# LikeLy-Journey/SegmenTron

Measured on AMD Instinct MI355X. Metric: images/sec fwd+bwd DeepLabv3+_xception65 @1025x2049, higher is better.
Workload: dtype bf16; 1 GPU; DeepLabv3+_xception65 train step (fwd + CE loss + bwd + SGD) @1025x2049, batch 2/GPU (BASELINE.json configs[2]); global_batch=2, bn=BN, parallelism=dp1, full_size=True

## Files before the change

include/segmentron_hip.h:

```cpp
#ifndef SEGMENTRON_HIP_H
#define SEGMENTRON_HIP_H
#ifdef __cplusplus
extern "C" {
#endif

const char* seg_last_error(void);
int seg_version(void);

int seg_conv_gemm_fwd(int dtype, const void* x, long ldx, int N, int Hi, int Wi, int C,
                      const void* w, int O, int KH, int KW, int stride, int pad, int dil,
                      int pro_mode, const float* pro_scale, const float* pro_shift,
                      const float* bias, void* y, long ldy, int Ho, int Wo, int out_H, int out_W,
                      int out_s, float* stat_partial, const void* ep_x, long ldep,
                      const float* ep_c0, const float* ep_c1, int tconv, void* stream);
int seg_conv_gemm_tiles_m(int N, int Ho, int Wo);

int seg_conv_gemm_wgrad(int dtype, const void* x, long ldx, int N, int Hi, int Wi, int C,
                        const void* dy, long lddy, int Ho, int Wo, int O, int KH, int KW,
                        int stride, int pad, int dil, int pro_mode, const float* pro_scale,
                        const float* pro_shift, float* partial, int splits, void* stream);
int seg_conv_gemm_stat_rows(int dtype, int N, int Ho, int Wo, int C, int O, int KH, int KW,
                            int stride, int pad, int dil, int tconv, int has_bias, int pro_mode);
int seg_conv_gemm_wgrad_splits(int dtype, int N, int Ho, int Wo, int C, int O, int KH, int KW,
                               int stride, int pad, int dil, int pro_mode);

int seg_dwconv3x3(int dtype, int mode, const void* x, long ldx, int N, int Hi, int Wi, int C,
                  const float* w9c, int w_layout, int stride, int dil, int pro_mode,
                  const float* pro_scale, const float* pro_shift, void* y, long ldy, int Ho, int Wo,
                  float* stat_partial, int grid_y, void* stream);
int seg_dwconv_grid_y(int dtype, int C, int N, int Ho, int Wo, int stride, int dil, int kind);
int seg_dwconv3x3_wgrad_finalize(const float* partial, int R, int C, float* dw_c9, void* stream);
int seg_dwconv3x3_wgrad(int dtype, const void* x, long ldx, int N, int Hi, int Wi, int C,
                        const void* dy, long lddy, int Ho, int Wo, int stride, int dil,
                        int pro_mode, const float* pro_scale, const float* pro_shift,
                        float* partial, int grid_y, void* stream);

int seg_dwconv3x3_bwd_fused(int dtype, const void* dy, long lddy, const void* x, long ldx, int N,
                            int H, int W, int C, const float* w9c, int w_layout, int dil,
                            int pro_mode, const float* pro_scale, const float* pro_shift, void* g,
                            long ldg, float* partial_w, float* partial_bn, int grid_y,
                            void* stream);
int seg_dwconv3x3_bwd_fused_add_ok(int dil);
int seg_dwconv3x3_bwd_fused_add(int dtype, const void* dy, long lddy, const void* x, long ldx, int N,
                                int H, int W, int C, const float* w9c, int w_layout, int pro_mode,
                                const float* pro_scale, const float* pro_shift, const void* res,
                                long ldr, void* g, long ldg, float* partial_w, float* partial_bn,
                                int grid_y, void* stream);

int seg_colsum(const float* in, long R, int L, double* out_d, float* out_f, double* ws,
               void* stream);
int seg_colsum_count(const float* in, long R, int L, double* out_d, double count, double* ws,
                     void* stream);
int seg_bn_finalize(const double* sums, double count, const double* count_dev,
                    const float* gamma, const float* beta, float eps, float momentum, float* running_mean, float* running_var,
                    float* mean, float* invstd, float* scale, float* shift, int C,
                    const float* mean_offset, void* stream);
int seg_bn_finalize_p(const float* partial, long R, double count, const float* gamma,
                      const float* beta, float eps, float momentum, float* running_mean,
                      float* running_var, float* mean, float* invstd, float* scale, float* shift,
                      int C, const float* mean_offset, double* ws, void* stream);
int seg_bn_finalize_small(int dtype, const void* y, long ldy, long M, int C, const float* gamma,
                          const float* beta, float eps, float momentum, float* running_mean,
                          float* running_var, float* mean, float* invstd, float* scale,
                          float* shift, const float* mean_offset, void* stream);
int seg_bn_moments_small(int dtype, const void* y, long ldy, long M, int C, double* moments,
                         void* stream);
int seg_bn_finalize_small_sync(void* p2p, int dtype, const void* y, long ldy, long M, int C,
                               const float* gamma, const float* beta, float eps, float momentum,
                               float* running_mean, float* running_var, float* mean, float* invstd,
                               float* scale, float* shift, const float* mean_offset,
                               double* count_out, void* stream);
int seg_sum_n(int dtype, int n, const void* const* xs, const long* lds, void* y, long ldy, long M,
              int C, void* stream);
int seg_bn_eval_affine(const float* gamma, const float* beta, const float* rm, const float* rv,
                       float eps, float* scale, float* shift, int C, void* stream);
int seg_bn_eval_affine_multi(int n, const float* const* gamma, const float* const* beta,
                             const float* const* rm, const float* const* rv, const float* eps,
                             float* const* out, const int* C, void* stream);
int seg_bn_apply(int dtype, const void* x, long ldx, int mode_x, const float* sx, const float* tx,
                 const void* r, long ldr, int mode_r, const float* sr, const float* tr,
                 const float* chan_mul, long rows_per_n, const void* elem_mul, long ldm,
                 int post_relu, void* y, long ldy, long M, int C, void* stream);
int seg_bn_bwd_grid_y(int dtype, int C, long M);
int seg_ew_geom_query(int dtype, int C, long M, int what);
int seg_bn_bwd_reduce(int dtype, const void* g, long ldg, const void* x, long ldx, int mode,
                      const float* scale, const float* shift, const float* chan_mul,
                      long rows_per_n, const void* elem_mul, long ldm, long M, int C,
                      float* partial, int grid_y, void* stream);
int seg_bn_bwd_small(int dtype, const void* g, long ldg, const void* x, long ldx, void* dx,
                     long lddx, long M, int C, int mode, const float* scale, const float* shift,
                     const float* mean, const float* invstd, const float* gamma,
                     const float* chan_mul, long rows_per_n, const void* elem_mul, long ldm,
                     double count, int training, float* dgamma, float* dbeta, void* stream);
int seg_bn_bwd_finalize(const double* sums, double count, const double* count_dev,
                        const float* mean, const float* invstd, const float* gamma, float* dgamma, float* dbeta, float* c0, float* c1,
                        int C, void* stream);
int seg_bn_bwd_finalize_s(const double* sums, double count, const double* count_dev,
                          const float* mean, const float* invstd, const float* gamma, float* dgamma,
                          float* dbeta, float* c0, float* c1, int C, double grad_scale, void* stream);
int seg_bn_bwd_finalize_p(const float* partial, long R, double count, const float* mean,
                          const float* invstd, const float* gamma, float* dgamma, float* dbeta,
                          float* c0, float* c1, int C, double* ws, void* stream);
int seg_dw_bwd_finalize(const float* partial_bn, int Rb, double count, const float* mean,
                        const float* invstd, const float* gamma, float* dgamma, float* dbeta,
                        float* c0, float* c1, const float* partial_w, int Rw, float* dw_c9, int C,
                        void* stream);
int seg_bn_bwd_apply(int dtype, const void* g, long ldg, const void* x, long ldx, int mode,
                     const float* scale, const float* shift, const float* c0, const float* c1,
                     const float* chan_mul, long rows_per_n, const void* elem_mul, long ldm,
                     void* dx, long lddx, long M, int C, void* stream);

int seg_gn_chunks(long HW);
int seg_gn_moments(int dtype, const void* u, long ldu, const void* v, long ldv, int N, long HW,
                   int C, float* partial, void* stream);
int seg_gn_fwd_finalize(const float* partial, int N, long HW, int C, int G, const float* gamma,
                        const float* beta, double eps, float* mean_rstd, float* coef,
                        void* stream);
int seg_gn_bwd_finalize(const float* partial, int N, long HW, int C, int G,
                        const float* mean_rstd, const float* gamma, float* coef, float* contrib,
                        void* stream);
int seg_gn_affine(int dtype, const void* u, long ldu, const void* v, long ldv, const float* coef,
                  void* out, long ldo, int N, long HW, int C, void* stream);

int seg_fold_weights(int dtype, const float* W, const float* scale, const float* shift, void* Wp,
                     void* WpT, float* bprime, int O, int C, void* stream);
int seg_fold_bwd_rows(int O);
int seg_fold_bwd_reduce(const float* W, const float* dWp, int splits, const float* scale,
                        const float* shift, const float* db, float* dW, float* dsdt, int O, int C,
                        void* stream);
int seg_fold_bwd_finalize(const float* dsdt, int rows, double count, const double* count_dev,
                          const float* mean, const float* invstd, const float* gamma, const float* scale, float* dgamma, float* dbeta,
                          float* c0, float* c1, int C, void* stream);
int seg_fold_bwd_finalize_s(const float* dsdt, int rows, double count, const double* count_dev,
                            const float* mean, const float* invstd, const float* gamma,
                            const float* scale, float* dgamma, float* dbeta, float* c0, float* c1,
                            int C, double grad_scale, void* stream);

int seg_maxpool_fwd(int dtype, const void* x, long ldx, int N, int Hi, int Wi, int C, int k,
                    int stride, int pad, int pro_mode, const float* pro_scale,
                    const float* pro_shift, void* y, long ldy, int Ho, int Wo, void* idx,
                    void* stream);
int seg_maxpool_bwd(int dtype, void* gx, long ldgx, int N, int Hi, int Wi, int C, int k, int stride,
                    int pad, const void* gy, long ldgy, int Ho, int Wo, const void* idx,
                    void* stream);
int seg_adaptive_avgpool_chunks(int H, int W, int o);
int seg_adaptive_avgpool_partial(int dtype, const void* x, long ldx, int N, int H, int W, int C,
                                 int o, float* partial, int chunks, void* stream);
int seg_adaptive_avgpool_bwd(int dtype, void* gx, long ldgx, int N, int H, int W, int C, int o,
                             const void* gy, long ldgy, void* stream);

int seg_bilinear_fwd(int dtype, const void* x, long ldx, int N, int Hi, int Wi, int C,
                     int pro_mode, const float* pro_scale, const float* pro_shift,
                     const float* chan_mul, void* y, long ldy, int Ho, int Wo, int align_corners,
                     void* stream);
int seg_bilinear_bwd(int dtype, void* gx, long ldgx, int N, int Hi, int Wi, int C, const void* gy,
                     long ldgy, int Ho, int Wo, int align_corners, void* stream);
int seg_nearest_add(int dtype, const void* x, long ldx, int mode_x, const float* sx,
                    const float* tx, const void* r, long ldr, int mode_r, const float* sr,
                    const float* tr, int shift, int post_relu, void* y, long ldy, int N, int H,
                    int W, int C, void* stream);
int seg_nearest_sum_bwd(int dtype, const void* g, long ldg, int N, int H, int W, int C, int shift,
                        void* gr, long ldgr, void* stream);
int seg_upsample_to_nchw(int dtype, const void* x, long ldx, int N, int Hi, int Wi, int C,
                         float* out, int Ho, int Wo, int align_corners, void* stream);
int seg_upsample_to_nchw_bwd(int dtype, void* gx, long ldgx, int N, int Hi, int Wi, int C,
                             const float* gy, int Ho, int Wo, int align_corners, void* stream);
int seg_nchw_to_nhwc_pad(int dtype, const float* x, int N, int Cin, int H, int W, void* y,
                         void* stream);

int seg_upsample_ce_blocks(int N, int H, int W);
int seg_upsample_ce_fwd(int dtype, const void* lo, long ld, int N, int Hi, int Wi, int C,
                        const long* target, int H, int W, long ignore_index, int align_corners,
                        double* ws, float* loss_out, void* stream);
int seg_upsample_ce_bwd(int dtype, const void* lo, long ld, int N, int Hi, int Wi, int C,
                        const long* target, int H, int W, long ignore_index, int align_corners,
                        const float* loss_out, const float* grad_out, void* dlo, long lddlo,
                        void* stream);

int seg_point_sample(int dtype_x, const void* x, long sn, long sp, long sc, int N, int H, int W,
                     int C, const float* pts, int P, int nearest, int dtype_y, void* y, long ldy,
                     int col, void* stream);
int seg_point_sample_bwd_ws(int N, int H, int W, int P);
int seg_point_sample_bwd(int dtype_g, const void* g, long ldg, int col, const float* pts, int N,
                         int P, int H, int W, int C, int dtype_x, void* dx, long lddx, int* ws,
                         void* stream);
int seg_point_uncertainty(int dtype, const void* x, long sn, long sp, long sc, int N, int H, int W,
                          int C, const float* pts, int P, float* u, void* stream);
int seg_point_topk_ws(int N, long L);
int seg_point_topk(const float* keys, int N, long L, int K, long* idx, int* ws, void* stream);
int seg_point_coords(const float* over, const long* idx, int N, int L, int K, const float* cover,
                     int P, int H, int W, float* pts, void* stream);
int seg_point_scatter(int dtype_r, const void* rend, long ldr, const long* idx, int N, int P,
                      int C, float* y, long sn, long sp, long sc, void* stream);
int seg_point_resize(int dtype, const void* x, long sn, long sp, long sc, int N, int Hi, int Wi,
                     int C, float* y, int Ho, int Wo, int align_corners, void* stream);
int seg_point_ce_blocks(long R);
int seg_point_ce_fwd(int dtype, const void* x, long ldx, long R, int C, const long* target,
                     long ignore_index, double* ws, float* loss_out, void* stream);
int seg_point_ce_bwd(int dtype, const void* x, long ldx, long R, int C, const long* target,
                     long ignore_index, const float* loss_out, const float* grad_out, void* dx,
                     long lddx, void* stream);

int seg_dwconv3x3_s2_grid_y(int C, int N, int H, int W);
int seg_dwconv3x3_s2_bwd_fused(int dtype, const void* dy, long lddy, const void* x, long ldx, int N,
                               int H, int W, int C, const float* w_c9, int pro_mode,
                               const float* pro_scale, const float* pro_shift, void* g, long ldg,
                               float* partial_w, float* partial_bn, int grid_y, void* stream);

int seg_sgd_multi_tensor(int ntensors, const void* const* params, const void* const* grads,
                         const void* const* bufs, const long* numel, const int* group,
                         const float* lr_dev, const float* wd_dev, float momentum, int first,
                         void* stream);
int seg_pack_multi(int dtype, int njobs, const void* const* srcs, const void* const* dsts,
                   const int* O, const int* C, const int* transpose, void* stream);

int seg_metric_update_nchw(const float* logits, int N, int C, int H, int W, const long* target,
                           int nclass, long* counters, void* stream);
int seg_metric_update_upsample(int dtype, const void* lo, long ld, int N, int Hi, int Wi, int C,
                               const long* target, int H, int W, int align_corners, int nclass,
                               long* counters, void* stream);

int seg_cca_attention(int dtype, const void* q, long ldq, const void* k, long ldk, int N, int H,
                      int W, int C, float* att, void* stream);
int seg_cca_attention_bwd(int dtype, const void* dout, long lddo, const void* v, long ldv, int N,
                          int H, int W, int C, const float* att, const float* scale, float* de,
                          void* stream);
int seg_cca_map(int dtype, const float* wt, const void* b, long ldb, int N, int H, int W, int C,
                int transposed, const float* gamma, const void* res, long ldres, void* out,
                long ldo, void* raw, long ldraw, void* stream);

int seg_row_softmax(const void* e, int dt_in, long lde, void* a, int dt_out, long lda, long R,
                    int L, int Lp, float sign, void* stream);
int seg_row_softmax_bwd(const void* a, int dt_a, long lda, const void* g, int dt_g, long ldg,
                        void* de, int dt_out, long ldde, long R, int L, int Lp, float sign,
                        void* stream);
int seg_p2p_create(int rank, int world, long slot_bytes, void** handle_out);
int seg_p2p_ipc_handle(void* handle, void* out64);
int seg_p2p_connect(void* handle, const void* handles);
int seg_p2p_all_reduce_f64(void* handle, void* buf, int n, void* stream);
int seg_p2p_all_reduce_f32(void* handle, void* buf, int n, void* stream);
int seg_p2p_status(void* handle);
int seg_p2p_set_timeout(void* handle, double seconds);
int seg_p2p_destroy(void* handle);
int seg_bn_finalize_p_sync(void* p2p, const float* partial, long R, double local_count,
                           const float* gamma, const float* beta, float eps, float momentum,
                           float* running_mean, float* running_var, float* mean, float* invstd,
                           float* scale, float* shift, int C, const float* mean_offset,
                           double* count_out, double* ws, void* stream);
int seg_bn_bwd_finalize_p_sync(void* p2p, const float* partial, long R, const double* count_dev,
                               const float* mean, const float* invstd, const float* gamma,
                               float* dgamma, float* dbeta, float* c0, float* c1, int C,
                               double grad_scale, double* ws, void* stream);
int seg_dw_bwd_finalize_sync(void* p2p, const float* partial_bn, int Rb, const double* count_dev,
                             const float* mean, const float* invstd, const float* gamma,
                             float* dgamma, float* dbeta, float* c0, float* c1,
                             const float* partial_w, int Rw, float* dw_c9, int C,
                             double grad_scale, void* stream);
int seg_fold_bwd_finalize_sync(void* p2p, const float* dsdt, int rows, const double* count_dev,
                               const float* mean, const float* invstd, const float* gamma,
                               const float* scale, float* dgamma, float* dbeta, float* c0,
                               float* c1, int C, double grad_scale, void* stream);

#ifdef __cplusplus
}
#endif
#endif
```

segmentron_amd/csrc/dwconv.hip:

```cpp
#include "common.h"
#include "dwconv_tiled.h"
#include "dwconv_slide.h"
#include <cstdlib>
#include <type_traits>

namespace seg {

constexpr bool g_dw_row = true;

constexpr int DW_TW = 4;
constexpr int DW_THREADS = 256;
enum { MODE_FWD = 0, MODE_DGRAD = 1 };

struct DwArgs {
  const void* x;
  const float* w;
  void* y;
  const float* pro_scale;
  const float* pro_shift;
  float* stat_partial;
  long ldx, ldy;
  int N, Hi, Wi, C;
  int Ho, Wo;
  int stride, pad, dil;
  int pro_mode;
  int cvb_log2;
  int CV;
  long strips;
};

__device__ __forceinline__ int fast_div(int s, int d, float inv) {
  int q = (int)((float)s * inv);
  if (q * d > s) --q;
  if ((q + 1) * d <= s) ++q;
  return q;
}

template <int VEC>
__device__ __forceinline__ void dw_act(float* f, int mode, const float* sc, const float* sh) {
  if (mode & PRO_AFFINE) {
#pragma unroll
    for (int i = 0; i < VEC; ++i) f[i] = fmaf(f[i], sc[i], sh[i]);
  }
  if (mode & PRO_RELU) {
#pragma unroll
    for (int i = 0; i < VEC; ++i) f[i] = fmaxf(f[i], 0.f);
  }
  if (mode & PRO_CLAMP6) {
#pragma unroll
    for (int i = 0; i < VEC; ++i) f[i] = fminf(f[i], 6.f);
  }
}

template <typename T, int MODE>
__global__ __launch_bounds__(DW_THREADS, 2) void dwconv_kernel(const DwArgs a) {
  using V = Vec<T>;
  constexpr int VEC = V::N;
  extern __shared__ __attribute__((aligned(16))) float dw_smem[];
  const int tid = threadIdx.x;
  const int cvb = 1 << a.cvb_log2;
  const int cx = tid & (cvb - 1), sy = tid >> a.cvb_log2;
  const int spb = DW_THREADS >> a.cvb_log2;
  const int cv = blockIdx.x * cvb + cx;
  const bool cok = cv < a.CV;
  const int c0 = cok ? cv * VEC : 0;
  const T* __restrict__ X = reinterpret_cast<const T*>(a.x);
  T* __restrict__ Y = reinterpret_cast<T*>(a.y);
  const int WQ = (a.Wo + DW_TW - 1) / DW_TW;
  const float inv_wq = 1.0f / (float)WQ, inv_ho = 1.0f / (float)a.Ho;

  float sc[VEC], sh[VEC];
  if (a.pro_mode & PRO_AFFINE) {
    load_params<VEC>(a.pro_scale, c0, sc);
    load_params<VEC>(a.pro_shift, c0, sh);
  } else {
#pragma unroll
    for (int i = 0; i < VEC; ++i) { sc[i] = 1.f; sh[i] = 0.f; }
  }
  float ssum[VEC], ssq[VEC];
#pragma unroll
  for (int i = 0; i < VEC; ++i) ssum[i] = ssq[i] = 0.f;

  const int nstrips = (int)a.strips;
  for (int s = blockIdx.y * spb + sy; s < nstrips; s += gridDim.y * spb) {
    if (!cok) continue;
    const int t = fast_div(s, WQ, inv_wq);
    const int wq = s - t * WQ;
    const int n = fast_div(t, a.Ho, inv_ho);
    const int ho = t - n * a.Ho;
    const int w0 = wq * DW_TW;
    float acc[DW_TW][VEC];
#pragma unroll
    for (int j = 0; j < DW_TW; ++j)
#pragma unroll
      for (int i = 0; i < VEC; ++i) acc[j][i] = 0.f;

#pragma unroll
    for (int kh = 0; kh < 3; ++kh) {
      int hi;
      if (MODE == MODE_FWD) {
        hi = ho * a.stride - a.pad + kh * a.dil;
      } else {
        const int hn = ho + a.pad - kh * a.dil;
        if (hn < 0 || (hn % a.stride) != 0) continue;
        hi = hn / a.stride;
      }
      if (hi < 0 || hi >= a.Hi) continue;
      const long rowbase = ((long)n * a.Hi + hi) * a.Wi;
#pragma unroll
      for (int kw = 0; kw < 3; ++kw) {
        float wv[VEC];
        load_params<VEC>(a.w + (kh * 3 + kw) * a.C, c0, wv);
#pragma unroll
        for (int j = 0; j < DW_TW; ++j) {
          const int wo = w0 + j;
          int wi;
          bool ok = wo < a.Wo;
          if (MODE == MODE_FWD) {
            wi = wo * a.stride - a.pad + kw * a.dil;
          } else {
            const int wn = wo + a.pad - kw * a.dil;
            ok = ok && wn >= 0 && (wn % a.stride) == 0;
            wi = wn / a.stride;
          }
          ok = ok && wi >= 0 && wi < a.Wi;
          if (ok) {
            float f[VEC];
            V::unpack_raw(V::load_raw(X + (rowbase + wi) * a.ldx + c0), f);
            dw_act<VEC>(f, a.pro_mode, sc, sh);
#pragma unroll
            for (int i = 0; i < VEC; ++i) acc[j][i] = fmaf(f[i], wv[i], acc[j][i]);
          }
        }
      }
    }
    const long orow = ((long)n * a.Ho + ho) * a.Wo;
#pragma unroll
    for (int j = 0; j < DW_TW; ++j) {
      if (w0 + j < a.Wo) {
        V::store(Y + (orow + w0 + j) * a.ldy + c0, acc[j]);
#pragma unroll
        for (int i = 0; i < VEC; ++i) {
          ssum[i] += acc[j][i];
          ssq[i] += acc[j][i] * acc[j][i];
        }
      }
    }
  }

  if (a.stat_partial != nullptr) {
    float* mine = dw_smem + ((long)sy * cvb + cx) * 2 * VEC;
#pragma unroll
    for (int i = 0; i < VEC; ++i) {
      mine[i] = ssum[i];
      mine[VEC + i] = ssq[i];
    }
    __syncthreads();
    for (int e = tid; e < cvb * 2 * VEC; e += DW_THREADS) {
      float tot = 0.f;
      for (int r = 0; r < spb; ++r) tot += dw_smem[(long)r * cvb * 2 * VEC + e];
      const int lcx = e / (2 * VEC), k = e % (2 * VEC);
      const int which = k / VEC, ci = k % VEC;
      const int c = (blockIdx.x * cvb + lcx) * VEC + ci;
      if (c < a.C) a.stat_partial[((long)blockIdx.y * 2 + which) * a.C + c] = tot;
    }
  }
}

struct DwWgradArgs {
  const void* x;
  const void* dy;
  float* partial;
  const float* pro_scale;
  const float* pro_shift;
  long ldx, lddy;
  int N, Hi, Wi, C, Ho, Wo;
  int stride, pad, dil;
  int pro_mode;
  int cvb_log2, CV;
  long strips;
};

template <typename T>
__global__ __launch_bounds__(DW_THREADS) void dwconv_wgrad_kernel(const DwWgradArgs a) {
  constexpr int VEC = Vec<T>::N;
  extern __shared__ __attribute__((aligned(16))) float dw_smem[];
  const int tid = threadIdx.x;
  const int cvb = 1 << a.cvb_log2;
  const int cx = tid & (cvb - 1), sy = tid >> a.cvb_log2;
  const int spb = DW_THREADS >> a.cvb_log2;
  const int cv = blockIdx.x * cvb + cx;
  const bool cok = cv < a.CV;
  const int c0 = cok ? cv * VEC : 0;
  const T* __restrict__ X = reinterpret_cast<const T*>(a.x);
  const T* __restrict__ DY = reinterpret_cast<const T*>(a.dy);
  const int WQ = (a.Wo + DW_TW - 1) / DW_TW;
  const float inv_wq = 1.0f / (float)WQ, inv_ho = 1.0f / (float)a.Ho;

  float sc[VEC], sh[VEC];
  if (a.pro_mode & PRO_AFFINE) {
    load_params<VEC>(a.pro_scale, c0, sc);
    load_params<VEC>(a.pro_shift, c0, sh);
  } else {
#pragma unroll
    for (int i = 0; i < VEC; ++i) { sc[i] = 1.f; sh[i] = 0.f; }
  }
  float acc[9][VEC];
#pragma unroll
  for (int k = 0; k < 9; ++k)
#pragma unroll
    for (int i = 0; i < VEC; ++i) acc[k][i] = 0.f;

  const int nstrips = (int)a.strips;
  for (int s = blockIdx.y * spb + sy; s < nstrips; s += gridDim.y * spb) {
    if (!cok) continue;
    const int t = fast_div(s, WQ, inv_wq);
    const int wq = s - t * WQ;
    const int n = fast_div(t, a.Ho, inv_ho);
    const int ho = t - n * a.Ho;
    const int w0 = wq * DW_TW;
    const long orow = ((long)n * a.Ho + ho) * a.Wo;
    float g[DW_TW][VEC];
#pragma unroll
    for (int j = 0; j < DW_TW; ++j) {
      const int wc = min(w0 + j, a.Wo - 1);
      Vec<T>::unpack(ldg16(DY + (orow + wc) * a.lddy + c0), g[j]);
      const float keep = (w0 + j < a.Wo) ? 1.f : 0.f;
#pragma unroll
      for (int i = 0; i < VEC; ++i) g[j][i] *= keep;
    }
#pragma unroll
    for (int kh = 0; kh < 3; ++kh) {
      const int hi = ho * a.stride - a.pad + kh * a.dil;
      if (hi < 0 || hi >= a.Hi) continue;
      const long rowbase = ((long)n * a.Hi + hi) * a.Wi;
#pragma unroll
      for (int kw = 0; kw < 3; ++kw) {
#pragma unroll
        for (int j = 0; j < DW_TW; ++j) {
          const int wi = (w0 + j) * a.stride - a.pad + kw * a.dil;
          if (w0 + j < a.Wo && wi >= 0 && wi < a.Wi) {
            float f[VEC];
            Vec<T>::unpack(ldg16(X + (rowbase + wi) * a.ldx + c0), f);
            dw_act<VEC>(f, a.pro_mode, sc, sh);
#pragma unroll
            for (int i = 0; i < VEC; ++i)
              acc[kh * 3 + kw][i] = fmaf(f[i], g[j][i], acc[kh * 3 + kw][i]);
          }
        }
      }
    }
  }
#pragma unroll
  for (int k3 = 0; k3 < 3; ++k3) {
    float* mine = dw_smem + ((long)sy * cvb + cx) * 3 * VEC;
#pragma unroll
    for (int kk = 0; kk < 3; ++kk)
#pragma unroll
      for (int i = 0; i < VEC; ++i) mine[kk * VEC + i] = acc[k3 * 3 + kk][i];
    __syncthreads();
    for (int e = tid; e < cvb * 3 * VEC; e += DW_THREADS) {
      float tot = 0.f;
      for (int r = 0; r < spb; ++r) tot += dw_smem[(long)r * cvb * 3 * VEC + e];
      const int lcx = e / (3 * VEC), k = e % (3 * VEC);
      const int kk = k / VEC, ci = k % VEC;
      const int c = (blockIdx.x * cvb + lcx) * VEC + ci;
      if (c < a.C) a.partial[((long)blockIdx.y * 9 + k3 * 3 + kk) * a.C + c] = tot;
    }
    __syncthreads();
  }
}

struct DwBwdArgs {
  const void* dy; const void* x; void* g;
  const float* w;
  const float* pro_scale; const float* pro_shift;
  float* partial_w;
  float* partial_bn;
  long lddy, ldx, ldg;
  int N, H, W, C, dil, pro_mode, cvb_log2, CV;
  long strips;
};

template <typename T>
__global__ __launch_bounds__(DW_THREADS) void dwconv_bwd_fused_kernel(const DwBwdArgs a) {
  constexpr int VEC = HVec<T>::N;
  extern __shared__ __attribute__((aligned(16))) float dw_smem[];
  const int tid = threadIdx.x;
  const int cvb = 1 << a.cvb_log2;
  const int cx = tid & (cvb - 1), sy = tid >> a.cvb_log2;
  const int spb = DW_THREADS >> a.cvb_log2;
  const int cv = blockIdx.x * cvb + cx;
  const bool cok = cv < a.CV;
  const int c0 = cok ? cv * VEC : 0;
  const T* __restrict__ DY = reinterpret_cast<const T*>(a.dy);
  const T* __restrict__ X = reinterpret_cast<const T*>(a.x);
  T* __restrict__ G = reinterpret_cast<T*>(a.g);
  const int WQ = (a.W + DW_TW - 1) / DW_TW;
  const float inv_wq = 1.0f / (float)WQ, inv_h = 1.0f / (float)a.H;
  const int d = a.dil;

  float sc[VEC], sh[VEC];
  if (a.pro_mode & PRO_AFFINE) {
    load_params<VEC>(a.pro_scale, c0, sc);
    load_params<VEC>(a.pro_shift, c0, sh);
  } else {
#pragma unroll
    for (int i = 0; i < VEC; ++i) { sc[i] = 1.f; sh[i] = 0.f; }
  }
  float accw[9][VEC], s1[VEC], s2[VEC];
#pragma unroll
  for (int k = 0; k < 9; ++k)
#pragma unroll
    for (int i = 0; i < VEC; ++i) accw[k][i] = 0.f;
#pragma unroll
  for (int i = 0; i < VEC; ++i) s1[i] = s2[i] = 0.f;

  const int nstrips = (int)a.strips;
  for (int s = blockIdx.y * spb + sy; s < nstrips; s += gridDim.y * spb) {
    if (!cok) continue;
    const int t = fast_div(s, WQ, inv_wq);
    const int wq = s - t * WQ;
    const int n = fast_div(t, a.H, inv_h);
    const int h = t - n * a.H;
    const int w0 = wq * DW_TW;
    const long prow = ((long)n * a.H + h) * a.W;
    float xr[DW_TW][VEC], xa[DW_TW][VEC], g[DW_TW][VEC];
#pragma unroll
    for (int j = 0; j < DW_TW; ++j) {
      const int wc = min(w0 + j, a.W - 1);
      HVec<T>::load(X + (prow + wc) * a.ldx + c0, xr[j]);
      const float keep = (w0 + j < a.W) ? 1.f : 0.f;
#pragma unroll
      for (int i = 0; i < VEC; ++i) {
        xa[j][i] = xr[j][i];
        g[j][i] = 0.f;
      }
      dw_act<VEC>(xa[j], a.pro_mode, sc, sh);
#pragma unroll
      for (int i = 0; i < VEC; ++i) {
        xa[j][i] *= keep;
        xr[j][i] *= keep;
      }
    }
#pragma unroll
    for (int kh = 0; kh < 3; ++kh) {
      const int r = h + (1 - kh) * d;
      if (r < 0 || r >= a.H) continue;
      const long rowbase = ((long)n * a.H + r) * a.W;
#pragma unroll
      for (int kw = 0; kw < 3; ++kw) {
        float wv[VEC];
        load_params<VEC>(a.w + (kh * 3 + kw) * a.C, c0, wv);
#pragma unroll
        for (int j = 0; j < DW_TW; ++j) {
          const int c = w0 + j + (1 - kw) * d;
          if (w0 + j < a.W && c >= 0 && c < a.W) {
            float dyv[VEC];
            HVec<T>::load(DY + (rowbase + c) * a.lddy + c0, dyv);
#pragma unroll
            for (int i = 0; i < VEC; ++i) {
              g[j][i] = fmaf(dyv[i], wv[i], g[j][i]);
              accw[kh * 3 + kw][i] = fmaf(dyv[i], xa[j][i], accw[kh * 3 + kw][i]);
            }
          }
        }
      }
    }
#pragma unroll
    for (int j = 0; j < DW_TW; ++j) {
      if (w0 + j < a.W) {
        if (a.pro_mode & PRO_RELU) {
#pragma unroll
          for (int i = 0; i < VEC; ++i) {
            const bool on = xa[j][i] > 0.f && (!(a.pro_mode & PRO_CLAMP6) || xa[j][i] < 6.f);
            g[j][i] = on ? g[j][i] : 0.f;
          }
        }
#pragma unroll
        for (int i = 0; i < VEC; ++i) {
          s1[i] += g[j][i];
          s2[i] = fmaf(g[j][i], xr[j][i], s2[i]);
        }
        HVec<T>::store(G + (prow + w0 + j) * a.ldg + c0, g[j]);
      }
    }
  }
#pragma unroll
  for (int k3 = 0; k3 < 4; ++k3) {
    if (k3 == 3 && a.partial_bn == nullptr) break;
    float* mine = dw_smem + ((long)sy * cvb + cx) * 3 * VEC;
#pragma unroll
    for (int kk = 0; kk < 3; ++kk)
#pragma unroll
      for (int i = 0; i < VEC; ++i)
        mine[kk * VEC + i] = k3 < 3 ? accw[(k3 < 3 ? k3 : 0) * 3 + kk][i]
                                    : (kk == 0 ? s1[i] : (kk == 1 ? s2[i] : 0.f));
    __syncthreads();
    const int ncol = (k3 < 3 ? 3 : 2) * VEC;
    for (int e = tid; e < cvb * 3 * VEC; e += DW_THREADS) {
      const int lcx = e / (3 * VEC), k = e % (3 * VEC);
      if (k >= ncol) continue;
      float tot = 0.f;
      for (int r = 0; r < spb; ++r) tot += dw_smem[(long)r * cvb * 3 * VEC + e];
      const int kk = k / VEC, ci = k % VEC;
      const int c = (blockIdx.x * cvb + lcx) * VEC + ci;
      if (c < a.C) {
        if (k3 < 3) a.partial_w[((long)blockIdx.y * 9 + k3 * 3 + kk) * a.C + c] = tot;
        else a.partial_bn[((long)blockIdx.y * 2 + kk) * a.C + c] = tot;
      }
    }
    __syncthreads();
  }
}

static int pick_cvb_log2(int CV) {
  int best = 5;
  double bu = 0;
  for (int l = 5; l >= 3; --l) {
    const int b = 1 << l;
    const double u = (double)CV / (double)(((CV + b - 1) / b) * b);
    if (u > bu + 1e-9) { bu = u; best = l; }
  }
  return best;
}

}

extern "C" int seg_dwconv_grid_y(int dtype, int C, int N, int Ho, int Wo, int stride, int dil,
                                 int kind) {
  using namespace seg;
  const int tiled_stride = kind == 0 ? stride : 1;
  if ((kind == 0 || kind == 1) && dw_slide_supported(stride, dil, C))
    return dw_slide_rows(C, N, Ho, Wo);
  if ((kind == 0 || stride == 1) && dw_tiled_supported(tiled_stride, dil))
    return dw_tiled_grid_y(dtype, C, N, Ho, Wo, kind);
  if (kind == 0 && stride == 2 && dil == 1)
    return dw_tiled_s2_grid_y(dtype, C, N, Ho, Wo);
  if (g_dw_row && (kind == 0 || kind == 1) && dw_row_supported(stride, dil) && C % 4 == 0)
    return dw_row_grid_y(dtype, C, N, Ho, Wo, dil);
  const int vec = dtype == DT_BF16 ? 8 : 4;
  const int CV = C / vec;
  const int l = pick_cvb_log2(CV);
  const int spb = DW_THREADS >> l;
  const long strips = (long)N * Ho * ((Wo + DW_TW - 1) / DW_TW);
  const int gx = (CV + (1 << l) - 1) >> l;
  long gy = (strips + spb - 1) / spb;
  long cap = 1536 / gx;
  if (cap < 1) cap = 1;
  if (gy > cap) gy = cap;
  return (int)gy;
}
extern "C" int seg_dwconv3x3(int dtype, int mode, const void* x, long ldx, int N, int Hi, int Wi,
                             int C, const float* w9c, int w_layout, int stride, int dil, int pro_mode,
                             const float* pro_scale, const float* pro_shift, void* y, long ldy,
                             int Ho, int Wo, float* stat_partial, int grid_y, void* stream) {
  using namespace seg;
  const int vec = dtype == DT_BF16 ? 8 : 4;
  SEG_REQUIRE(dtype == DT_F32 || dtype == DT_BF16, "dwconv3x3: bad dtype %d", dtype);
  SEG_REQUIRE(C % vec == 0 && ldx % vec == 0 && ldy % vec == 0,
              "dwconv3x3: C/ldx/ldy must be multiples of %d", vec);
  SEG_REQUIRE(((pro_mode & PRO_AFFINE) == 0) || (pro_scale && pro_shift),
              "dwconv3x3: affine prologue without scale/shift");
  SEG_REQUIRE(mode == MODE_FWD || stat_partial == nullptr, "dwconv3x3: stats only in forward");
  SEG_REQUIRE(grid_y >= 1, "dwconv3x3: grid_y must be >= 1");
  if (mode == MODE_FWD && dw_slide_supported(stride, dil, C)) {
    SEG_REQUIRE(Ho == Hi && Wo == Wi, "dwconv3x3: stride 1 keeps the size");
    return launch_dw_slide_fwd(dtype, x, ldx, N, Hi, Wi, C, w9c, w_layout, pro_mode, pro_scale,
                               pro_shift, y, ldy, stat_partial, grid_y, (hipStream_t)stream);
  }
  if (mode == MODE_FWD && dw_tiled_supported(stride, dil)) {
    SEG_REQUIRE(Ho == Hi && Wo == Wi, "dwconv3x3: stride 1 keeps the size");
    return launch_dw_tiled(dtype, x, ldx, N, Hi, Wi, C, w9c, w_layout, dil, pro_mode, pro_scale,
                           pro_shift, y, ldy, stat_partial, grid_y, (hipStream_t)stream);
  }
  if (mode == MODE_FWD && stride == 2 && dil == 1) {
    SEG_REQUIRE(Ho == (Hi + 1) / 2 && Wo == (Wi + 1) / 2, "dwconv3x3: stride-2 output size");
    SEG_REQUIRE((long)N * Hi * Wi < (1L << 31), "dwconv3x3: tensor exceeds 32-bit pixel offsets");
    return launch_dw_tiled_s2(dtype, x, ldx, N, Hi, Wi, C, w9c, w_layout, pro_mode, pro_scale,
                              pro_shift, y, ldy, stat_partial, grid_y, (hipStream_t)stream);
  }
  SEG_REQUIRE(w_layout == 0, "dwconv3x3: the strip kernels take tap-major [9][C] weights");
  if (g_dw_row && mode == MODE_FWD && dw_row_supported(stride, dil) && C % 4 == 0) {
    SEG_REQUIRE(Ho == Hi && Wo == Wi, "dwconv3x3: stride 1 keeps the size");
    return launch_dw_row_fwd(dtype, x, ldx, N, Hi, Wi, C, w9c, dil, pro_mode, pro_scale, pro_shift,
                             y, ldy, stat_partial, grid_y, (hipStream_t)stream);
  }
  DwArgs a;
  a.x = x; a.w = w9c; a.y = y; a.pro_scale = pro_scale; a.pro_shift = pro_shift;
  a.stat_partial = stat_partial; a.ldx = ldx; a.ldy = ldy;
  a.N = N; a.Hi = Hi; a.Wi = Wi; a.C = C; a.Ho = Ho; a.Wo = Wo;
  a.stride = stride; a.pad = dil; a.dil = dil; a.pro_mode = pro_mode;
  const int kvec = vec;
  a.CV = C / kvec; a.cvb_log2 = pick_cvb_log2(a.CV);
  a.strips = (long)N * Ho * ((Wo + DW_TW - 1) / DW_TW);
  const int gx = (a.CV + (1 << a.cvb_log2) - 1) >> a.cvb_log2;
  SEG_REQUIRE(grid_y >= 1, "dwconv3x3: grid_y must be >= 1");
  const dim3 grid(gx, grid_y);
  const size_t lds = stat_partial ? (size_t)DW_THREADS * 2 * kvec * sizeof(float) : 0;
  hipStream_t st = (hipStream_t)stream;
  SEG_REQUIRE(a.strips < (1L << 31), "dwconv3x3: too many strips");
  SEG_REQUIRE((long)N * Hi * Wi * ldx < (1L << 31), "dwconv3x3: tensor exceeds 32-bit offsets");
#define SEG_DW_LAUNCH(TT, MM) \
  hipLaunchKernelGGL((dwconv_kernel<TT, MM>), grid, dim3(DW_THREADS), lds, st, a)
  if (dtype == DT_BF16) {
    if (mode == MODE_FWD) SEG_DW_LAUNCH(bf16_t, MODE_FWD); else SEG_DW_LAUNCH(bf16_t, MODE_DGRAD);
  } else {
    if (mode == MODE_FWD) SEG_DW_LAUNCH(float, MODE_FWD); else SEG_DW_LAUNCH(float, MODE_DGRAD);
  }
#undef SEG_DW_LAUNCH
  return check_launch("dwconv3x3");
}

extern "C" int seg_dwconv3x3_wgrad(int dtype, const void* x, long ldx, int N, int Hi, int Wi,
                                   int C, const void* dy, long lddy, int Ho, int Wo, int stride,
                                   int dil, int pro_mode, const float* pro_scale,
                                   const float* pro_shift, float* partial, int grid_y,
                                   void* stream) {
  using namespace seg;
  const int vec = dtype == DT_BF16 ? 8 : 4;
  SEG_REQUIRE(dtype == DT_F32 || dtype == DT_BF16, "dwconv3x3_wgrad: bad dtype %d", dtype);
  SEG_REQUIRE(C % vec == 0 && ldx % vec == 0 && lddy % vec == 0,
              "dwconv3x3_wgrad: C/ldx/lddy must be multiples of %d", vec);
  SEG_REQUIRE(grid_y >= 1, "dwconv3x3_wgrad: grid_y must be >= 1");
  if (dw_tiled_supported(stride, dil)) {
    SEG_REQUIRE(Ho == Hi && Wo == Wi, "dwconv3x3_wgrad: stride 1 keeps the size");
    return launch_dw_wgrad_tiled(dtype, x, ldx, N, Hi, Wi, C, dy, lddy, dil, pro_mode, pro_scale,
                                 pro_shift, partial, grid_y, (hipStream_t)stream);
  }
  DwWgradArgs a;
  a.x = x; a.dy = dy; a.partial = partial; a.pro_scale = pro_scale; a.pro_shift = pro_shift;
  a.ldx = ldx; a.lddy = lddy; a.N = N; a.Hi = Hi; a.Wi = Wi; a.C = C; a.Ho = Ho; a.Wo = Wo;
  a.stride = stride; a.pad = dil; a.dil = dil; a.pro_mode = pro_mode;
  a.CV = C / vec; a.cvb_log2 = pick_cvb_log2(a.CV);
  a.strips = (long)N * Ho * ((Wo + DW_TW - 1) / DW_TW);
  const int gx = (a.CV + (1 << a.cvb_log2) - 1) >> a.cvb_log2;
  SEG_REQUIRE(grid_y >= 1, "dwconv3x3_wgrad: grid_y must be >= 1");
  const dim3 grid(gx, grid_y);
  const size_t lds = (size_t)DW_THREADS * 3 * vec * sizeof(float);
  hipStream_t st = (hipStream_t)stream;
  SEG_REQUIRE(a.strips < (1L << 31), "dwconv3x3_wgrad: too many strips");
  if (dtype == DT_BF16)
    hipLaunchKernelGGL((dwconv_wgrad_kernel<bf16_t>), grid, dim3(DW_THREADS), lds, st, a);
  else
    hipLaunchKernelGGL((dwconv_wgrad_kernel<float>), grid, dim3(DW_THREADS), lds, st, a);
  return check_launch("dwconv3x3_wgrad");
}

extern "C" int seg_dwconv3x3_bwd_fused_add_ok(int dil) { return dil == 1 ? 1 : 0; }

extern "C" int seg_dwconv3x3_bwd_fused_add(int dtype, const void* dy, long lddy, const void* x,
                                           long ldx, int N, int H, int W, int C, const float* w9c,
                                           int w_layout, int pro_mode, const float* pro_scale,
                                           const float* pro_shift, const void* res, long ldr,
                                           void* g, long ldg, float* partial_w, float* partial_bn,
                                           int grid_y, void* stream) {
  using namespace seg;
  SEG_REQUIRE(dtype == DT_F32 || dtype == DT_BF16, "dwconv3x3_bwd_fused_add: bad dtype %d", dtype);
  const int tvec = dtype == DT_BF16 ? 8 : 4;
  SEG_REQUIRE(C % tvec == 0 && ldx % tvec == 0 && lddy % tvec == 0 && ldg % tvec == 0 &&
                  ldr % 4 == 0 && res != nullptr,
              "dwconv3x3_bwd_fused_add: C/ld must be multiples of %d, res non-null", tvec);
  SEG_REQUIRE(((pro_mode & PRO_AFFINE) == 0) || (pro_scale && pro_shift),
              "dwconv3x3_bwd_fused_add: affine prologue without scale/shift");
  SEG_REQUIRE(grid_y >= 1 && partial_w != nullptr, "dwconv3x3_bwd_fused_add: bad grid/partials");
  if (dw_slide_supported(1, 1, C))
    return launch_dw_slide_bwd(dtype, dy, lddy, x, ldx, N, H, W, C, w9c, w_layout, pro_mode,
                               pro_scale, pro_shift, g, ldg, partial_w, partial_bn, grid_y,
                               (hipStream_t)stream, res, ldr);
  return launch_dw_bwd_tiled(dtype, dy, lddy, x, ldx, N, H, W, C, w9c, w_layout, 1, pro_mode,
                             pro_scale, pro_shift, g, ldg, partial_w, partial_bn, grid_y,
                             (hipStream_t)stream, res, ldr);
}

extern "C" int seg_dwconv3x3_bwd_fused(int dtype, const void* dy, long lddy, const void* x,
                                       long ldx, int N, int H, int W, int C, const float* w9c,
                                       int w_layout, int dil, int pro_mode, const float* pro_scale,
                                       const float* pro_shift, void* g, long ldg,
                                       float* partial_w, float* partial_bn, int grid_y,
                                       void* stream) {
  using namespace seg;
  const int vec = 4;
  SEG_REQUIRE(dtype == DT_F32 || dtype == DT_BF16, "dwconv3x3_bwd_fused: bad dtype %d", dtype);
  SEG_REQUIRE(C % vec == 0 && ldx % vec == 0 && lddy % vec == 0 && ldg % vec == 0,
              "dwconv3x3_bwd_fused: C/ld must be multiples of %d", vec);
  SEG_REQUIRE(((pro_mode & PRO_AFFINE) == 0) || (pro_scale && pro_shift),
              "dwconv3x3_bwd_fused: affine prologue without scale/shift");
  SEG_REQUIRE(grid_y >= 1 && partial_w != nullptr, "dwconv3x3_bwd_fused: bad grid/partials");
  if (dw_slide_supported(1, dil, C))
    return launch_dw_slide_bwd(dtype, dy, lddy, x, ldx, N, H, W, C, w9c, w_layout, pro_mode,
                               pro_scale, pro_shift, g, ldg, partial_w, partial_bn, grid_y,
                               (hipStream_t)stream);
  if (dw_tiled_supported(1, dil)) {
    const int tvec = dtype == DT_BF16 ? 8 : 4;
    SEG_REQUIRE(C % tvec == 0 && ldx % tvec == 0 && lddy % tvec == 0 && ldg % tvec == 0,
                "dwconv3x3_bwd_fused: C/ld must be multiples of %d", tvec);
    return launch_dw_bwd_tiled(dtype, dy, lddy, x, ldx, N, H, W, C, w9c, w_layout, dil, pro_mode,
                               pro_scale, pro_shift, g, ldg, partial_w, partial_bn, grid_y,
                               (hipStream_t)stream);
  }
  SEG_REQUIRE(w_layout == 0, "dwconv3x3_bwd_fused: the strip kernel takes tap-major weights");
  if (g_dw_row && dw_row_supported(1, dil))
    return launch_dw_row_bwd(dtype, dy, lddy, x, ldx, N, H, W, C, w9c, dil, pro_mode, pro_scale,
                             pro_shift, g, ldg, partial_w, partial_bn, grid_y, (hipStream_t)stream);
  DwBwdArgs a;
  a.dy = dy; a.x = x; a.g = g; a.w = w9c; a.pro_scale = pro_scale; a.pro_shift = pro_shift;
  a.partial_w = partial_w; a.partial_bn = partial_bn;
  a.lddy = lddy; a.ldx = ldx; a.ldg = ldg; a.N = N; a.H = H; a.W = W; a.C = C; a.dil = dil;
  a.pro_mode = pro_mode; a.CV = C / vec; a.cvb_log2 = pick_cvb_log2(a.CV);
  a.strips = (long)N * H * ((W + DW_TW - 1) / DW_TW);
  SEG_REQUIRE(a.strips < (1L << 31), "dwconv3x3_bwd_fused: too many strips");
  SEG_REQUIRE((long)N * H * W * lddy < (1L << 31), "dwconv3x3_bwd_fused: 32-bit offsets");
  const int gx = (a.CV + (1 << a.cvb_log2) - 1) >> a.cvb_log2;
  const dim3 grid(gx, grid_y);
  const size_t lds = (size_t)DW_THREADS * 3 * vec * sizeof(float);
  hipStream_t st = (hipStream_t)stream;
  if (dtype == DT_BF16)
    hipLaunchKernelGGL((dwconv_bwd_fused_kernel<bf16_t>), grid, dim3(DW_THREADS), lds, st, a);
  else
    hipLaunchKernelGGL((dwconv_bwd_fused_kernel<float>), grid, dim3(DW_THREADS), lds, st, a);
  return check_launch("dwconv3x3_bwd_fused");
}

extern "C" int seg_dwconv3x3_wgrad_finalize(const float* partial, int R, int C, float* dw_c9,
                                            void* stream) {
  using namespace seg;
  SEG_REQUIRE(R >= 1 && C >= 1, "dwconv3x3_wgrad_finalize: bad R/C");
  return launch_dw_wgrad_finalize(partial, R, C, dw_c9, (hipStream_t)stream);
}
```

segmentron_amd/csrc/dwconv_slide.h:

```cpp
#pragma once
#include <hip/hip_runtime.h>

namespace seg {
bool dw_slide_supported(int stride, int dil, int C);
int dw_slide_rows(int C, int N, int H, int W);
int launch_dw_slide_fwd(int dtype, const void* x, long ldx, int N, int H, int W, int C,
                        const float* w, int w_layout, int pro_mode, const float* sc,
                        const float* sh, void* y, long ldy, float* stat_partial, int rows,
                        hipStream_t st);
int launch_dw_slide_bwd(int dtype, const void* dy, long lddy, const void* x, long ldx, int N, int H,
                        int W, int C, const float* w, int w_layout, int pro_mode, const float* sc,
                        const float* sh, void* g, long ldg, float* partial_w, float* partial_bn,
                        int rows, hipStream_t st, const void* res = nullptr, long ldr = 0);
}
```

segmentron_amd/csrc/dwconv_slide.hip:

```cpp
#include <type_traits>
#include "common.h"
#include "dwconv_slide.h"

namespace seg {

constexpr int SL_THREADS = 256, SL_CQ = 16, SL_WL = 16;
constexpr int SL_DEPTH_F = 2, SL_OCC_F = 4, SL_DEPTH_B = 2;
#define SL_SCHED_BARRIER() __builtin_amdgcn_sched_barrier(0)

struct DwSlideArgs {
  const void* x;
  const void* dy;
  const void* res;
  void* y;
  const float* w;
  int w_layout;
  const float* sc; const float* sh;
  float* partial;
  float* partial_bn;
  long ldx, lddy, ldy, ldr;
  int N, H, W, C, pro_mode, rs, nstrips, nwblk, ncblk;
};

struct SlBlock { int n, strip, wblk, cblk, prow; };
__device__ __forceinline__ SlBlock sl_block(const DwSlideArgs& a) {
  const int nblk = a.ncblk * a.nwblk * a.nstrips * a.N;
  int L = xcd_remap(blockIdx.x, nblk);
  SlBlock b;
  b.cblk = L % a.ncblk;
  L /= a.ncblk;
  b.prow = L;
  b.wblk = L % a.nwblk;
  L /= a.nwblk;
  b.strip = L % a.nstrips;
  b.n = L / a.nstrips;
  return b;
}

typedef float f32x2 __attribute__((ext_vector_type(2)));
typedef short s16x2 __attribute__((ext_vector_type(2)));
struct Q4 { f32x2 lo, hi; };
__device__ __forceinline__ Q4 q4_zero() { Q4 q; q.lo = q.hi = (f32x2){0.f, 0.f}; return q; }
__device__ __forceinline__ void q4_fma(Q4& acc, const Q4& a, const Q4& b) {
  acc.lo = __builtin_elementwise_fma(a.lo, b.lo, acc.lo);
  acc.hi = __builtin_elementwise_fma(a.hi, b.hi, acc.hi);
}
template <typename T> struct SlIO;
template <> struct SlIO<bf16_t> {
  typedef uint2 raw_t;
  static constexpr int BYTES = 8;
  __device__ static __forceinline__ Q4 unpack(const raw_t& r) {
    Q4 q;
    q.lo = (f32x2){__uint_as_float(r.x << 16), __uint_as_float(r.x & 0xFFFF0000u)};
    q.hi = (f32x2){__uint_as_float(r.y << 16), __uint_as_float(r.y & 0xFFFF0000u)};
    return q;
  }
  __device__ static __forceinline__ raw_t relu_raw(const raw_t& r) {
    const s16x2 z = {0, 0};
    raw_t o;
    o.x = __builtin_bit_cast(unsigned, __builtin_elementwise_max(__builtin_bit_cast(s16x2, r.x), z));
    o.y = __builtin_bit_cast(unsigned, __builtin_elementwise_max(__builtin_bit_cast(s16x2, r.y), z));
    return o;
  }
  static constexpr bool RAW_RELU = true;
  __device__ static __forceinline__ raw_t pack(const Q4& q) {
    return make_uint2(pack_bf16x2(q.lo.x, q.lo.y), pack_bf16x2(q.hi.x, q.hi.y));
  }
};
template <> struct SlIO<float> {
  typedef uint4 raw_t;
  static constexpr int BYTES = 16;
  __device__ static __forceinline__ Q4 unpack(const raw_t& r) {
    Q4 q;
    q.lo = (f32x2){__uint_as_float(r.x), __uint_as_float(r.y)};
    q.hi = (f32x2){__uint_as_float(r.z), __uint_as_float(r.w)};
    return q;
  }
  __device__ static __forceinline__ raw_t relu_raw(const raw_t& r) { return r; }
  static constexpr bool RAW_RELU = false;
  __device__ static __forceinline__ raw_t pack(const Q4& q) {
    return make_uint4(__float_as_uint(q.lo.x), __float_as_uint(q.lo.y), __float_as_uint(q.hi.x),
                      __float_as_uint(q.hi.y));
  }
};
template <typename R>
__device__ __forceinline__ R sl_ld(const unsigned char* __restrict__ base, unsigned off) {
  return *reinterpret_cast<const R*>(base + off);
}
template <typename R>
__device__ __forceinline__ void sl_st(unsigned char* __restrict__ base, unsigned off, const R& v) {
  *reinterpret_cast<R*>(base + off) = v;
}

__device__ __forceinline__ void sl_load_taps(const DwSlideArgs& a, int c, Q4 (&wt)[9]) {
  float f[36];
  if (a.w_layout & 1) {
    const float4* p = reinterpret_cast<const float4*>(a.w + (long)c * 9);
#pragma unroll
    for (int j = 0; j < 9; ++j) {
      const float4 v = p[j];
      f[4 * j] = v.x; f[4 * j + 1] = v.y; f[4 * j + 2] = v.z; f[4 * j + 3] = v.w;
    }
#pragma unroll
    for (int k = 0; k < 9; ++k) {
      const int tap = (a.w_layout & 2) ? 8 - k : k;
      wt[k].lo = (f32x2){(a.w_layout & 2) ? f[8 - k] : f[k], (a.w_layout & 2) ? f[9 + 8 - k] : f[9 + k]};
      wt[k].hi = (f32x2){(a.w_layout & 2) ? f[18 + 8 - k] : f[18 + k],
                         (a.w_layout & 2) ? f[27 + 8 - k] : f[27 + k]};
      (void)tap;
    }
  } else {
#pragma unroll
    for (int k = 0; k < 9; ++k) {
      const int tap = (a.w_layout & 2) ? 8 - k : k;
      const float4 v = *reinterpret_cast<const float4*>(a.w + (long)tap * a.C + c);
      wt[k].lo = (f32x2){v.x, v.y};
      wt[k].hi = (f32x2){v.z, v.w};
    }
  }
}

template <int MODE, bool RELU_DONE>
__device__ __forceinline__ void sl_act(Q4& q, const Q4& sc, const Q4& sh) {
  const f32x2 z = {0.f, 0.f}, six = {6.f, 6.f};
  if (MODE & PRO_AFFINE) {
    q.lo = __builtin_elementwise_fma(q.lo, sc.lo, sh.lo);
    q.hi = __builtin_elementwise_fma(q.hi, sc.hi, sh.hi);
  }
  if ((MODE & PRO_RELU) && !RELU_DONE) {
    q.lo = __builtin_elementwise_max(q.lo, z);
    q.hi = __builtin_elementwise_max(q.hi, z);
  }
  if (MODE & PRO_CLAMP6) {
    q.lo = __builtin_elementwise_min(q.lo, six);
    q.hi = __builtin_elementwise_min(q.hi, six);
  }
}

struct SlThread {
  int c, w, r0, r1, rlast;
  bool live, lm, rm;
  unsigned off_m, off_0, off_p;
  bool edge, first, last;
  unsigned off_e;
  int bp_up, bp_dn;
};
template <int ESIZE>
__device__ __forceinline__ SlThread sl_thread(const DwSlideArgs& a, const SlBlock& b, long ld) {
  const int tid = threadIdx.x, cq = tid & (SL_CQ - 1), wl = tid >> 4;
  SlThread t;
  const int cfull = (b.cblk * SL_CQ + cq) * 4, wfull = b.wblk * SL_WL + wl;
  t.c = min(cfull, a.C - 4);
  t.w = min(wfull, a.W - 1);
  t.live = wfull < a.W && cfull < a.C;
  t.lm = t.w >= 1;
  t.rm = t.w + 1 < a.W;
  t.r0 = b.strip * a.rs;
  t.r1 = min(a.H, t.r0 + a.rs);
  t.rlast = min(t.r1, a.H - 1);
  t.off_m = (unsigned)((max(t.w - 1, 0) * ld + t.c) * ESIZE);
  t.off_0 = (unsigned)((t.w * ld + t.c) * ESIZE);
  t.off_p = (unsigned)((min(t.w + 1, a.W - 1) * ld + t.c) * ESIZE);
  const int lane = tid & 63, col = lane >> 4;
  t.first = col == 0;
  t.last = col == 3;
  t.edge = t.first || t.last;
  t.off_e = t.first ? t.off_m : (t.last ? t.off_p : 0xFFFFFFFFu);
  t.bp_up = ((lane - 16) & 63) * 4;
  t.bp_dn = ((lane + 16) & 63) * 4;
  return t;
}

typedef unsigned int sl_u32x2 __attribute__((ext_vector_type(2)));
typedef unsigned int sl_u32x4 __attribute__((ext_vector_type(4)));
template <typename R> __device__ __forceinline__ R sl_ld_edge(const unsigned char* row, unsigned nbytes, unsigned off);
template <> __device__ __forceinline__ uint2 sl_ld_edge<uint2>(const unsigned char* row, unsigned nbytes, unsigned off) {
  const __amdgpu_buffer_rsrc_t r = __builtin_amdgcn_make_buffer_rsrc((void*)row, 0, (int)nbytes, 0x00020000);
  const sl_u32x2 v = __builtin_amdgcn_raw_buffer_load_b64(r, (int)off, 0, 0);
  return make_uint2(v.x, v.y);
}
template <> __device__ __forceinline__ uint4 sl_ld_edge<uint4>(const unsigned char* row, unsigned nbytes, unsigned off) {
  const __amdgpu_buffer_rsrc_t r = __builtin_amdgcn_make_buffer_rsrc((void*)row, 0, (int)nbytes, 0x00020000);
  const sl_u32x4 v = __builtin_amdgcn_raw_buffer_load_b128(r, (int)off, 0, 0);
  return make_uint4(v.x, v.y, v.z, v.w);
}
template <typename R> __device__ __forceinline__ void sl_st_row(unsigned char* row, unsigned nbytes, unsigned off, const R& v);
template <> __device__ __forceinline__ void sl_st_row<uint2>(unsigned char* row, unsigned nbytes, unsigned off, const uint2& v) {
  const __amdgpu_buffer_rsrc_t r = __builtin_amdgcn_make_buffer_rsrc((void*)row, 0, (int)nbytes, 0x00020000);
  const sl_u32x2 d = {v.x, v.y};
  __builtin_amdgcn_raw_buffer_store_b64(d, r, (int)off, 0, 0);
}
template <> __device__ __forceinline__ void sl_st_row<uint4>(unsigned char* row, unsigned nbytes, unsigned off, const uint4& v) {
  const __amdgpu_buffer_rsrc_t r = __builtin_amdgcn_make_buffer_rsrc((void*)row, 0, (int)nbytes, 0x00020000);
  const sl_u32x4 d = {v.x, v.y, v.z, v.w};
  __builtin_amdgcn_raw_buffer_store_b128(d, r, (int)off, 0, 0);
}
template <typename R> __device__ __forceinline__ R sl_bperm(int addr, const R& v);
template <> __device__ __forceinline__ uint2 sl_bperm<uint2>(int addr, const uint2& v) {
  return make_uint2((unsigned)__builtin_amdgcn_ds_bpermute(addr, (int)v.x),
                    (unsigned)__builtin_amdgcn_ds_bpermute(addr, (int)v.y));
}
template <> __device__ __forceinline__ uint4 sl_bperm<uint4>(int addr, const uint4& v) {
  return make_uint4((unsigned)__builtin_amdgcn_ds_bpermute(addr, (int)v.x),
                    (unsigned)__builtin_amdgcn_ds_bpermute(addr, (int)v.y),
                    (unsigned)__builtin_amdgcn_ds_bpermute(addr, (int)v.z),
                    (unsigned)__builtin_amdgcn_ds_bpermute(addr, (int)v.w));
}
__device__ __forceinline__ uint2 sl_sel(bool c, const uint2& a, const uint2& b) {
  return make_uint2(c ? a.x : b.x, c ? a.y : b.y);
}
__device__ __forceinline__ uint4 sl_sel(bool c, const uint4& a, const uint4& b) {
  return make_uint4(c ? a.x : b.x, c ? a.y : b.y, c ? a.z : b.z, c ? a.w : b.w);
}
template <typename R>
__device__ __forceinline__ void sl_neighbours(const SlThread& t, const R (&raw)[3], R& left, R& right) {
  const R up = sl_bperm<R>(t.bp_up, raw[0]), dn = sl_bperm<R>(t.bp_dn, raw[0]);
  left = sl_sel(t.first, raw[1], up);
  right = sl_sel(t.last, raw[1], dn);
}

template <typename T, int MODE, bool XCHG>
__global__ __launch_bounds__(SL_THREADS, SL_OCC_F) void dwconv_slide_fwd_kernel(const DwSlideArgs a) {
  using IO = SlIO<T>;
  using raw_t = typename IO::raw_t;
  constexpr int ES = sizeof(T);
  constexpr bool RAWRELU = IO::RAW_RELU && MODE == PRO_RELU;
  const int tid = threadIdx.x, cq = tid & (SL_CQ - 1);
  const SlBlock b = sl_block(a);
  const SlThread t = sl_thread<ES>(a, b, a.ldx);
  const int r0 = t.r0, r1 = t.r1;

  Q4 wt[9], sc, sh;
  sc = sh = q4_zero();
  const unsigned char* __restrict__ Xb = reinterpret_cast<const unsigned char*>(a.x) +
                                         (long)b.n * a.H * a.W * a.ldx * ES;
  unsigned char* __restrict__ Yb = reinterpret_cast<unsigned char*>(a.y) +
                                   (long)b.n * a.H * a.W * a.ldy * ES;
  const long xpitch = (long)a.W * a.ldx * ES, ypitch = (long)a.W * a.ldy * ES;
  const unsigned rowbytes = (unsigned)xpitch;
  const unsigned yoff = t.live ? (unsigned)((t.w * a.ldy + t.c) * ES) : 0xFFFFFFFFu;

  auto issue = [&](int r, raw_t (&raw)[3]) {
    const unsigned char* __restrict__ row = Xb + (long)min(max(r, 0), t.rlast) * xpitch;
    if (XCHG) {
      raw[0] = sl_ld<raw_t>(row, t.off_0);
      raw[1] = sl_ld_edge<raw_t>(row, rowbytes, t.off_e);
    } else {
      raw[0] = sl_ld<raw_t>(row, t.off_0);
      raw[1] = sl_ld<raw_t>(row, t.off_m);
      raw[2] = sl_ld<raw_t>(row, t.off_p);
    }
  };
  auto commit = [&](int r, const raw_t (&raw)[3], Q4 (&row)[3], auto check) {
    constexpr bool CHECK = decltype(check)::value;
    const bool rv = !CHECK || (r >= 0 && r < a.H);
    raw_t r3[3];
    r3[1] = raw[0];
    if (XCHG) {
      sl_neighbours<raw_t>(t, raw, r3[0], r3[2]);
    } else {
      r3[0] = raw[1];
      r3[2] = raw[2];
    }
#pragma unroll
    for (int k = 0; k < 3; ++k) {
      row[k] = IO::unpack(RAWRELU ? IO::relu_raw(r3[k]) : r3[k]);
      sl_act<MODE, RAWRELU>(row[k], sc, sh);
      if (CHECK && !rv) row[k] = q4_zero();
    }
  };
  Q4 ssum = q4_zero(), ssq = q4_zero();
  auto compute = [&](int ro, const Q4 (&ra)[3], const Q4 (&rb)[3], const Q4 (&rc)[3]) {
    Q4 acc = q4_zero();
#pragma unroll
    for (int kw = 0; kw < 3; ++kw) q4_fma(acc, ra[kw], wt[kw]);
#pragma unroll
    for (int kw = 0; kw < 3; ++kw) q4_fma(acc, rb[kw], wt[3 + kw]);
#pragma unroll
    for (int kw = 0; kw < 3; ++kw) q4_fma(acc, rc[kw], wt[6 + kw]);
    sl_st_row<raw_t>(Yb + (long)ro * ypitch, (unsigned)ypitch, yoff, IO::pack(acc));
    ssum.lo += acc.lo; ssum.hi += acc.hi;
    q4_fma(ssq, acc, acc);
  };

  constexpr int D = SL_DEPTH_F, U = (D % 3 == 0) ? D : 3 * D;
  Q4 win[3][3];
  raw_t ring[D][3];
#pragma unroll
  for (int j = 0; j < D; ++j) issue(r0 - 1 + j, ring[j]);
  sl_load_taps(a, t.c, wt);
  if (MODE & PRO_AFFINE) {
    const float4 s4 = *reinterpret_cast<const float4*>(a.sc + t.c);
    const float4 t4 = *reinterpret_cast<const float4*>(a.sh + t.c);
    sc.lo = (f32x2){s4.x, s4.y}; sc.hi = (f32x2){s4.z, s4.w};
    sh.lo = (f32x2){t4.x, t4.y}; sh.hi = (f32x2){t4.z, t4.w};
  }
#pragma unroll
  for (int kh = 0; kh < 3; ++kh) {
    if (!t.lm) wt[kh * 3] = q4_zero();
    if (!t.rm) wt[kh * 3 + 2] = q4_zero();
  }
  commit(r0 - 1, ring[0], win[0], std::true_type{});
  issue(r0 - 1 + D, ring[0]);
  commit(r0, ring[1 % D], win[1], std::false_type{});
  issue(r0 + D, ring[1 % D]);
  int ro = r0;
  for (; ro + U < r1; ro += U) {
#pragma unroll
    for (int k = 0; k < U; ++k) {
      commit(ro + k + 1, ring[(k + 2) % D], win[(k + 2) % 3], std::false_type{});
      issue(ro + k + 1 + D, ring[(k + 2) % D]);
      SL_SCHED_BARRIER();
      compute(ro + k, win[k % 3], win[(k + 1) % 3], win[(k + 2) % 3]);
      SL_SCHED_BARRIER();
    }
  }
#pragma unroll
  for (int k = 0; k < U; ++k) {
    if (ro + k < r1) {
      commit(ro + k + 1, ring[(k + 2) % D], win[(k + 2) % 3], std::true_type{});
      issue(ro + k + 1 + D, ring[(k + 2) % D]);
      compute(ro + k, win[k % 3], win[(k + 1) % 3], win[(k + 2) % 3]);
    }
  }

  if (a.partial != nullptr) {
    __shared__ float red[4][SL_CQ][8];
    float v[8] = {ssum.lo.x, ssum.lo.y, ssum.hi.x, ssum.hi.y, ssq.lo.x, ssq.lo.y, ssq.hi.x, ssq.hi.y};
#pragma unroll
    for (int i = 0; i < 8; ++i) {
      v[i] = t.live ? v[i] : 0.f;
      v[i] += __shfl_xor(v[i], 16, 64);
      v[i] += __shfl_xor(v[i], 32, 64);
    }
    if ((tid & 63) < SL_CQ) {
#pragma unroll
      for (int i = 0; i < 8; ++i) red[tid >> 6][cq][i] = v[i];
    }
    __syncthreads();
    if (tid < SL_CQ * 8) {
      const int q = tid >> 3, k = tid & 7;
      const float tot = red[0][q][k] + red[1][q][k] + red[2][q][k] + red[3][q][k];
      const int ch = (b.cblk * SL_CQ + q) * 4 + (k & 3);
      if (ch < a.C) a.partial[((long)b.prow * 2 + (k >> 2)) * a.C + ch] = tot;
    }
  }
}

template <typename T, int MODE, bool RES, bool XCHG>
__global__ __launch_bounds__(SL_THREADS, 2) void dwconv_slide_bwd_kernel(const DwSlideArgs a) {
  using IO = SlIO<T>;
  using raw_t = typename IO::raw_t;
  constexpr int ES = sizeof(T);
  const int tid = threadIdx.x, cq = tid & (SL_CQ - 1);
  const SlBlock b = sl_block(a);
  const SlThread t = sl_thread<ES>(a, b, a.lddy);
  const int r0 = t.r0, r1 = t.r1;

  Q4 wt[9], sc, sh;
  sc = sh = q4_zero();
  const long img = (long)b.n * a.H * a.W;
  const unsigned char* __restrict__ Db = reinterpret_cast<const unsigned char*>(a.dy) + img * a.lddy * ES;
  const unsigned char* __restrict__ Xb = reinterpret_cast<const unsigned char*>(a.x) + img * a.ldx * ES;
  const unsigned char* __restrict__ Rb =
      RES ? reinterpret_cast<const unsigned char*>(a.res) + img * a.ldr * ES : nullptr;
  unsigned char* __restrict__ Gb = reinterpret_cast<unsigned char*>(a.y) + img * a.ldy * ES;
  const long dpitch = (long)a.W * a.lddy * ES, xpitch = (long)a.W * a.ldx * ES;
  const long rpitch = (long)a.W * a.ldr * ES, gpitch = (long)a.W * a.ldy * ES;
  const unsigned rowbytes = (unsigned)dpitch;
  const unsigned xoff = (unsigned)((t.w * a.ldx + t.c) * ES), roff = (unsigned)((t.w * a.ldr + t.c) * ES);
  const unsigned goff = t.live ? (unsigned)((t.w * a.ldy + t.c) * ES) : 0xFFFFFFFFu;

  auto issue = [&](int r, raw_t (&raw)[3]) {
    const unsigned char* __restrict__ row = Db + (long)min(max(r, 0), t.rlast) * dpitch;
    if (XCHG) {
      raw[0] = sl_ld<raw_t>(row, t.off_0);
      raw[1] = sl_ld_edge<raw_t>(row, rowbytes, t.off_e);
    } else {
      raw[0] = sl_ld<raw_t>(row, t.off_0);
      raw[1] = sl_ld<raw_t>(row, t.off_m);
      raw[2] = sl_ld<raw_t>(row, t.off_p);
    }
  };
  auto issue_x = [&](int r, raw_t& xr, raw_t& rr) {
    const int rcl = min(r, r1 - 1);
    xr = sl_ld<raw_t>(Xb + (long)rcl * xpitch, xoff);
    if (RES) rr = sl_ld<raw_t>(Rb + (long)rcl * rpitch, roff);
  };
  auto commit = [&](int r, const raw_t (&raw)[3], Q4 (&row)[3], auto check) {
    constexpr bool CHECK = decltype(check)::value;
    const bool rv = !CHECK || (r >= 0 && r < a.H);
    raw_t r3[3];
    r3[1] = raw[0];
    if (XCHG) {
      sl_neighbours<raw_t>(t, raw, r3[0], r3[2]);
    } else {
      r3[0] = raw[1];
      r3[2] = raw[2];
    }
#pragma unroll
    for (int k = 0; k < 3; ++k) {
      row[k] = IO::unpack(r3[k]);
      if (CHECK && !rv) row[k] = q4_zero();
    }
  };
  Q4 accw[9], s1 = q4_zero(), s2 = q4_zero();
#pragma unroll
  for (int k = 0; k < 9; ++k) accw[k] = q4_zero();

  auto compute = [&](int ro, const raw_t& xraw, const raw_t& rraw, const Q4 (&ra)[3],
                     const Q4 (&rb)[3], const Q4 (&rcw)[3]) {
    const Q4 xr = IO::unpack(xraw);
    Q4 xa = xr;
    sl_act<MODE, false>(xa, sc, sh);
    Q4 g = q4_zero();
#pragma unroll
    for (int bq = 0; bq < 3; ++bq) { q4_fma(g, ra[bq], wt[8 - bq]); q4_fma(accw[8 - bq], ra[bq], xa); }
#pragma unroll
    for (int bq = 0; bq < 3; ++bq) { q4_fma(g, rb[bq], wt[5 - bq]); q4_fma(accw[5 - bq], rb[bq], xa); }
#pragma unroll
    for (int bq = 0; bq < 3; ++bq) { q4_fma(g, rcw[bq], wt[2 - bq]); q4_fma(accw[2 - bq], rcw[bq], xa); }
    if (MODE & PRO_RELU) {
      auto on = [&](float v) { return v > 0.f && (!(MODE & PRO_CLAMP6) || v < 6.f); };
      g.lo.x = on(xa.lo.x) ? g.lo.x : 0.f; g.lo.y = on(xa.lo.y) ? g.lo.y : 0.f;
      g.hi.x = on(xa.hi.x) ? g.hi.x : 0.f; g.hi.y = on(xa.hi.y) ? g.hi.y : 0.f;
    }
    if (RES) {
      const Q4 rr = IO::unpack(rraw);
      Q4 o;
      o.lo = g.lo + rr.lo;
      o.hi = g.hi + rr.hi;
      sl_st_row<raw_t>(Gb + (long)ro * gpitch, (unsigned)gpitch, goff, IO::pack(o));
    } else {
      sl_st_row<raw_t>(Gb + (long)ro * gpitch, (unsigned)gpitch, goff, IO::pack(g));
    }
    s1.lo += g.lo; s1.hi += g.hi;
    q4_fma(s2, g, xr);
  };

  constexpr int D = SL_DEPTH_B, U = (D % 3 == 0) ? D : 3 * D;
  Q4 win[3][3];
  raw_t ring[D][3], xring[D], rring[D];
#pragma unroll
  for (int j = 0; j < D; ++j) {
    issue(r0 - 1 + j, ring[j]);
    rring[j] = xring[j] = sl_ld<raw_t>(Xb + (long)min(r0 + j, r1 - 1) * xpitch, xoff);
    if (RES) rring[j] = sl_ld<raw_t>(Rb + (long)min(r0 + j, r1 - 1) * rpitch, roff);
  }
  sl_load_taps(a, t.c, wt);
  if (MODE & PRO_AFFINE) {
    const float4 s4 = *reinterpret_cast<const float4*>(a.sc + t.c);
    const float4 t4 = *reinterpret_cast<const float4*>(a.sh + t.c);
    sc.lo = (f32x2){s4.x, s4.y}; sc.hi = (f32x2){s4.z, s4.w};
    sh.lo = (f32x2){t4.x, t4.y}; sh.hi = (f32x2){t4.z, t4.w};
  }
#pragma unroll
  for (int kh = 0; kh < 3; ++kh) {
    if (!t.lm) wt[kh * 3 + 2] = q4_zero();
    if (!t.rm) wt[kh * 3] = q4_zero();
  }
  commit(r0 - 1, ring[0], win[0], std::true_type{});
  issue(r0 - 1 + D, ring[0]);
  commit(r0, ring[1 % D], win[1], std::false_type{});
  issue(r0 + D, ring[1 % D]);
  int ro = r0;
  for (; ro + U < r1; ro += U) {
#pragma unroll
    for (int k = 0; k < U; ++k) {
      commit(ro + k + 1, ring[(k + 2) % D], win[(k + 2) % 3], std::false_type{});
      issue(ro + k + 1 + D, ring[(k + 2) % D]);
      const raw_t xraw = xring[k % D], rraw = rring[k % D];
      issue_x(ro + k + D, xring[k % D], rring[k % D]);
      SL_SCHED_BARRIER();
      compute(ro + k, xraw, rraw, win[k % 3], win[(k + 1) % 3], win[(k + 2) % 3]);
      SL_SCHED_BARRIER();
    }
  }
#pragma unroll
  for (int k = 0; k < U; ++k) {
    if (ro + k < r1) {
      commit(ro + k + 1, ring[(k + 2) % D], win[(k + 2) % 3], std::true_type{});
      issue(ro + k + 1 + D, ring[(k + 2) % D]);
      const raw_t xraw = xring[k % D], rraw = rring[k % D];
      issue_x(ro + k + D, xring[k % D], rring[k % D]);
      compute(ro + k, xraw, rraw, win[k % 3], win[(k + 1) % 3], win[(k + 2) % 3]);
    }
  }

  float v[44];
#pragma unroll
  for (int k = 0; k < 9; ++k) {
    const int kw = k % 3;
    const bool keep = t.live && (kw != 2 || t.lm) && (kw != 0 || t.rm);
    v[k * 4] = keep ? accw[k].lo.x : 0.f; v[k * 4 + 1] = keep ? accw[k].lo.y : 0.f;
    v[k * 4 + 2] = keep ? accw[k].hi.x : 0.f; v[k * 4 + 3] = keep ? accw[k].hi.y : 0.f;
  }
  v[36] = s1.lo.x; v[37] = s1.lo.y; v[38] = s1.hi.x; v[39] = s1.hi.y;
  v[40] = s2.lo.x; v[41] = s2.lo.y; v[42] = s2.hi.x; v[43] = s2.hi.y;
#pragma unroll
  for (int i = 36; i < 44; ++i) v[i] = t.live ? v[i] : 0.f;
#pragma unroll
  for (int i = 0; i < 44; ++i) {
    v[i] += __shfl_xor(v[i], 16, 64);
    v[i] += __shfl_xor(v[i], 32, 64);
  }
  __shared__ float red[4][SL_CQ][44];
  if ((tid & 63) < SL_CQ) {
#pragma unroll
    for (int i = 0; i < 44; ++i) red[tid >> 6][cq][i] = v[i];
  }
  __syncthreads();
  for (int e = tid; e < SL_CQ * 44; e += SL_THREADS) {
    const int q = e / 44, k = e - q * 44;
    const float tot = red[0][q][k] + red[1][q][k] + red[2][q][k] + red[3][q][k];
    const int ch = (b.cblk * SL_CQ + q) * 4 + (k & 3), r = k >> 2;
    if (ch < a.C) {
      if (r < 9) a.partial[((long)b.prow * 9 + r) * a.C + ch] = tot;
      else if (a.partial_bn != nullptr) a.partial_bn[((long)b.prow * 2 + (r - 9)) * a.C + ch] = tot;
    }
  }
}

bool dw_slide_supported(int stride, int dil, int C) { return stride == 1 && dil == 1 && C % 4 == 0; }

static void slide_geom(DwSlideArgs& a, int N, int H, int W, int C) {
  a.ncblk = (C / 4 + SL_CQ - 1) / SL_CQ;
  a.nwblk = (W + SL_WL - 1) / SL_WL;
  long ns = (H + 21) / 43;
  const long per_strip = (long)N * a.nwblk * a.ncblk;
  const long want = (400 + per_strip - 1) / per_strip;
  if (ns < want) ns = want;
  if (ns > H / 8) ns = H / 8;
  const long cap = 1024 / ((long)N * a.nwblk);
  if (ns > cap) ns = cap;
  if (ns < 1) ns = 1;
  a.rs = (int)((H + ns - 1) / ns);
  a.nstrips = (H + a.rs - 1) / a.rs;
}

int dw_slide_rows(int C, int N, int H, int W) {
  DwSlideArgs a;
  slide_geom(a, N, H, W, C);
  return N * a.nstrips * a.nwblk;
}

static bool slide_exchange(const DwSlideArgs& a, int esize) {
  return (long)a.N * a.H * a.W * a.C * esize >= (30L << 20);
}
template <typename T>
static void slide_launch_fwd(const DwSlideArgs& a, dim3 grid, hipStream_t st) {
  const bool xc = slide_exchange(a, (int)sizeof(T));
  switch (a.pro_mode) {
#define SL_CASE(M)                                                                                  \
  case M:                                                                                           \
    if (xc) hipLaunchKernelGGL((dwconv_slide_fwd_kernel<T, M, true>), grid, dim3(SL_THREADS), 0, st, a);  \
    else hipLaunchKernelGGL((dwconv_slide_fwd_kernel<T, M, false>), grid, dim3(SL_THREADS), 0, st, a);    \
    break;
    SL_CASE(0) SL_CASE(1) SL_CASE(2) SL_CASE(3) SL_CASE(5) SL_CASE(7)
#undef SL_CASE
    default: break;
  }
}
template <typename T, bool RES>
static void slide_launch_bwd(const DwSlideArgs& a, dim3 grid, hipStream_t st) {
  const bool xc = slide_exchange(a, (int)sizeof(T));
  switch (a.pro_mode) {
#define SL_CASE(M)                                                                                       \
  case M:                                                                                                \
    if (xc) hipLaunchKernelGGL((dwconv_slide_bwd_kernel<T, M, RES, true>), grid, dim3(SL_THREADS), 0, st, a);  \
    else hipLaunchKernelGGL((dwconv_slide_bwd_kernel<T, M, RES, false>), grid, dim3(SL_THREADS), 0, st, a);    \
    break;
    SL_CASE(0) SL_CASE(1) SL_CASE(2) SL_CASE(3) SL_CASE(5) SL_CASE(7)
#undef SL_CASE
    default: break;
  }
}
static bool slide_mode_ok(int m) { return m == 0 || m == 1 || m == 2 || m == 3 || m == 5 || m == 7; }

int launch_dw_slide_fwd(int dtype, const void* x, long ldx, int N, int H, int W, int C,
                        const float* w, int w_layout, int pro_mode, const float* sc,
                        const float* sh, void* y, long ldy, float* stat_partial, int rows,
                        hipStream_t st) {
  DwSlideArgs a;
  a.x = x; a.dy = nullptr; a.res = nullptr; a.y = y; a.w = w; a.w_layout = w_layout;
  a.sc = sc; a.sh = sh; a.partial = stat_partial; a.partial_bn = nullptr;
  a.ldx = ldx; a.lddy = 0; a.ldy = ldy; a.ldr = 0;
  a.N = N; a.H = H; a.W = W; a.C = C; a.pro_mode = pro_mode;
  slide_geom(a, N, H, W, C);
  SEG_REQUIRE(slide_mode_ok(pro_mode), "dwconv (slide): unsupported prologue mode %d", pro_mode);
  SEG_REQUIRE(C % 4 == 0 && ldx % 4 == 0 && ldy % 4 == 0,
              "dwconv (slide): C/ldx/ldy must be multiples of 4");
  SEG_REQUIRE(stat_partial == nullptr || rows == N * a.nstrips * a.nwblk,
              "dwconv (slide): %d partial rows, the launch writes %d (seg_dwconv_grid_y)", rows,
              N * a.nstrips * a.nwblk);
  const dim3 grid((unsigned)((long)a.ncblk * a.nwblk * a.nstrips * N));
  if (dtype == DT_BF16) slide_launch_fwd<bf16_t>(a, grid, st);
  else slide_launch_fwd<float>(a, grid, st);
  return check_launch("dwconv3x3 (slide)");
}

int launch_dw_slide_bwd(int dtype, const void* dy, long lddy, const void* x, long ldx, int N, int H,
                        int W, int C, const float* w, int w_layout, int pro_mode, const float* sc,
                        const float* sh, void* g, long ldg, float* partial_w, float* partial_bn,
                        int rows, hipStream_t st, const void* res, long ldr) {
  DwSlideArgs a;
  a.x = x; a.dy = dy; a.res = res; a.y = g; a.w = w; a.w_layout = w_layout & 1;
  a.sc = sc; a.sh = sh; a.partial = partial_w; a.partial_bn = partial_bn;
  a.ldx = ldx; a.lddy = lddy; a.ldy = ldg; a.ldr = ldr;
  a.N = N; a.H = H; a.W = W; a.C = C; a.pro_mode = pro_mode;
  slide_geom(a, N, H, W, C);
  SEG_REQUIRE(slide_mode_ok(pro_mode), "dwconv bwd (slide): unsupported prologue mode %d", pro_mode);
  SEG_REQUIRE(C % 4 == 0 && ldx % 4 == 0 && lddy % 4 == 0 && ldg % 4 == 0 &&
                  (res == nullptr || ldr % 4 == 0),
              "dwconv bwd (slide): C/ldx/lddy/ldg/ldr must be multiples of 4");
  SEG_REQUIRE(rows == N * a.nstrips * a.nwblk,
              "dwconv bwd (slide): %d partial rows, the launch writes %d (seg_dwconv_grid_y)", rows,
              N * a.nstrips * a.nwblk);
  const dim3 grid((unsigned)((long)a.ncblk * a.nwblk * a.nstrips * N));
  if (dtype == DT_BF16) {
    if (res) slide_launch_bwd<bf16_t, true>(a, grid, st);
    else slide_launch_bwd<bf16_t, false>(a, grid, st);
  } else {
    if (res) slide_launch_bwd<float, true>(a, grid, st);
    else slide_launch_bwd<float, false>(a, grid, st);
  }
  return check_launch("dwconv3x3_bwd_fused (slide)");
}

}
```

segmentron_amd/csrc/resize.hip:

```cpp
#include "common.h"
#include "resize_taps.h"

namespace seg {

constexpr int RS_THREADS = 256;

struct ResizeArgs {
  const void* x; void* y;
  const float* scale; const float* shift; const float* chan_mul;
  long ldx, ldy;
  int N, Hi, Wi, Ho, Wo, C, CV;
  int mode, align;
  float sh, sw;
};

template <typename T>
__global__ __launch_bounds__(RS_THREADS) void bilinear_fwd_kernel(const ResizeArgs a) {
  constexpr int VEC = Vec<T>::N;
  const T* __restrict__ X = reinterpret_cast<const T*>(a.x);
  T* __restrict__ Y = reinterpret_cast<T*>(a.y);
  const long total = (long)a.N * a.Ho * a.Wo * a.CV;
  for (long i = (long)blockIdx.x * RS_THREADS + threadIdx.x; i < total;
       i += (long)gridDim.x * RS_THREADS) {
    const int cv = (int)(i % a.CV);
    long p = i / a.CV;
    const int wo = (int)(p % a.Wo); p /= a.Wo;
    const int ho = (int)(p % a.Ho);
    const int n = (int)(p / a.Ho);
    const int c0 = cv * VEC;
    int h0, h1, w0, w1; float lh, lw;
    taps(a.sh, ho, a.Hi, a.align, h0, h1, lh);
    taps(a.sw, wo, a.Wi, a.align, w0, w1, lw);
    const long base = (long)n * a.Hi * a.Wi;
    float f00[VEC], f01[VEC], f10[VEC], f11[VEC];
    Vec<T>::unpack(ldg16(X + (base + (long)h0 * a.Wi + w0) * a.ldx + c0), f00);
    Vec<T>::unpack(ldg16(X + (base + (long)h0 * a.Wi + w1) * a.ldx + c0), f01);
    Vec<T>::unpack(ldg16(X + (base + (long)h1 * a.Wi + w0) * a.ldx + c0), f10);
    Vec<T>::unpack(ldg16(X + (base + (long)h1 * a.Wi + w1) * a.ldx + c0), f11);
    apply_prologue<VEC>(f00, a.mode, a.scale, a.shift, c0);
    apply_prologue<VEC>(f01, a.mode, a.scale, a.shift, c0);
    apply_prologue<VEC>(f10, a.mode, a.scale, a.shift, c0);
    apply_prologue<VEC>(f11, a.mode, a.scale, a.shift, c0);
    float o[VEC];
#pragma unroll
    for (int k = 0; k < VEC; ++k) {
      const float top = (1.f - lw) * f00[k] + lw * f01[k];
      const float bot = (1.f - lw) * f10[k] + lw * f11[k];
      o[k] = (1.f - lh) * top + lh * bot;
    }
    if (a.chan_mul) {
      const float* m = a.chan_mul + (long)n * a.C + c0;
#pragma unroll
      for (int k = 0; k < VEC; ++k) o[k] *= m[k];
    }
    stg16(Y + (((long)n * a.Ho + ho) * a.Wo + wo) * a.ldy + c0, Vec<T>::pack(o));
  }
}

template <typename T>
__global__ __launch_bounds__(RS_THREADS) void bilinear_bwd_kernel(const ResizeArgs a) {
  constexpr int VEC = Vec<T>::N;
  const T* __restrict__ GY = reinterpret_cast<const T*>(a.y);
  T* __restrict__ GX = reinterpret_cast<T*>(const_cast<void*>(a.x));
  const long total = (long)a.N * a.Hi * a.Wi * a.CV;
  for (long i = (long)blockIdx.x * RS_THREADS + threadIdx.x; i < total;
       i += (long)gridDim.x * RS_THREADS) {
    const int cv = (int)(i % a.CV);
    long p = i / a.CV;
    const int wi = (int)(p % a.Wi); p /= a.Wi;
    const int hi = (int)(p % a.Hi);
    const int n = (int)(p / a.Hi);
    const int c0 = cv * VEC;
    int hlo, hhi, wlo, whi;
    cand_range(a.sh, hi, a.Ho, a.align, hlo, hhi);
    cand_range(a.sw, wi, a.Wo, a.align, wlo, whi);
    float acc[VEC];
#pragma unroll
    for (int k = 0; k < VEC; ++k) acc[k] = 0.f;
    for (int ho = hlo; ho <= hhi; ++ho) {
      const float wh = tap_weight(a.sh, ho, a.Hi, a.align, hi);
      if (wh == 0.f) continue;
      for (int wo = wlo; wo <= whi; ++wo) {
        const float ww = tap_weight(a.sw, wo, a.Wi, a.align, wi);
        if (ww == 0.f) continue;
        float g[VEC];
        Vec<T>::unpack(ldg16(GY + (((long)n * a.Ho + ho) * a.Wo + wo) * a.ldy + c0), g);
        const float w = wh * ww;
#pragma unroll
        for (int k = 0; k < VEC; ++k) acc[k] = fmaf(w, g[k], acc[k]);
      }
    }
    stg16(GX + (((long)n * a.Hi + hi) * a.Wi + wi) * a.ldx + c0, Vec<T>::pack(acc));
  }
}

constexpr int RSW_CVB = 8, RSW_PL = RS_THREADS / RSW_CVB;
template <typename T>
__global__ __launch_bounds__(RS_THREADS) void bilinear_bwd_wide_kernel(const ResizeArgs a) {
  constexpr int VEC = Vec<T>::N;
  __shared__ float red[RSW_PL][RSW_CVB][VEC];
  const T* __restrict__ GY = reinterpret_cast<const T*>(a.y);
  T* __restrict__ GX = reinterpret_cast<T*>(const_cast<void*>(a.x));
  const int cvb = (a.CV + RSW_CVB - 1) / RSW_CVB;
  const int cx = threadIdx.x & (RSW_CVB - 1), pl = threadIdx.x / RSW_CVB;
  long p = blockIdx.x / cvb;
  const int cv = (int)(blockIdx.x - p * cvb) * RSW_CVB + cx;
  const int wi = (int)(p % a.Wi); p /= a.Wi;
  const int hi = (int)(p % a.Hi);
  const int n = (int)(p / a.Hi);
  const bool cok = cv < a.CV;
  const int c0 = (cok ? cv : 0) * VEC;
  int hlo, hhi, wlo, whi;
  cand_range(a.sh, hi, a.Ho, a.align, hlo, hhi);
  cand_range(a.sw, wi, a.Wo, a.align, wlo, whi);
  const int nw = whi - wlo + 1, nf = (hhi - hlo + 1) * nw;
  float acc[VEC];
#pragma unroll
  for (int k = 0; k < VEC; ++k) acc[k] = 0.f;
  for (int f = pl; f < nf; f += RSW_PL) {
    const int r = f / nw;
    const int ho = hlo + r, wo = wlo + (f - r * nw);
    const float w = tap_weight(a.sh, ho, a.Hi, a.align, hi) * tap_weight(a.sw, wo, a.Wi, a.align, wi);
    if (w == 0.f || !cok) continue;
    float g[VEC];
    Vec<T>::unpack(ldg16(GY + (((long)n * a.Ho + ho) * a.Wo + wo) * a.ldy + c0), g);
#pragma unroll
    for (int k = 0; k < VEC; ++k) acc[k] = fmaf(w, g[k], acc[k]);
  }
#pragma unroll
  for (int k = 0; k < VEC; ++k) red[pl][cx][k] = acc[k];
  __syncthreads();
  if (pl == 0 && cok) {
    float tot[VEC];
#pragma unroll
    for (int k = 0; k < VEC; ++k) tot[k] = 0.f;
    for (int q = 0; q < RSW_PL; ++q)
#pragma unroll
      for (int k = 0; k < VEC; ++k) tot[k] += red[q][cx][k];
    stg16(GX + (((long)n * a.Hi + hi) * a.Wi + wi) * a.ldx + c0, Vec<T>::pack(tot));
  }
}

template <typename T>
__global__ __launch_bounds__(RS_THREADS) void upsample_to_nchw_kernel(const ResizeArgs a,
                                                                      float* __restrict__ out) {
  constexpr int VEC = Vec<T>::N;
  const T* __restrict__ X = reinterpret_cast<const T*>(a.x);
  const long total = (long)a.N * a.Ho * a.Wo;
  const long plane = (long)a.Ho * a.Wo;
  for (long i = (long)blockIdx.x * RS_THREADS + threadIdx.x; i < total;
       i += (long)gridDim.x * RS_THREADS) {
    long p = i;
    const int wo = (int)(p % a.Wo); p /= a.Wo;
    const int ho = (int)(p % a.Ho);
    const int n = (int)(p / a.Ho);
    int h0, h1, w0, w1; float lh, lw;
    taps(a.sh, ho, a.Hi, a.align, h0, h1, lh);
    taps(a.sw, wo, a.Wi, a.align, w0, w1, lw);
    const long base = (long)n * a.Hi * a.Wi;
    float* o = out + (long)n * a.C * plane + (long)ho * a.Wo + wo;
    for (int cv = 0; cv < a.CV; ++cv) {
      const int c0 = cv * VEC;
      float f00[VEC], f01[VEC], f10[VEC], f11[VEC];
      Vec<T>::unpack(ldg16(X + (base + (long)h0 * a.Wi + w0) * a.ldx + c0), f00);
      Vec<T>::unpack(ldg16(X + (base + (long)h0 * a.Wi + w1) * a.ldx + c0), f01);
      Vec<T>::unpack(ldg16(X + (base + (long)h1 * a.Wi + w0) * a.ldx + c0), f10);
      Vec<T>::unpack(ldg16(X + (base + (long)h1 * a.Wi + w1) * a.ldx + c0), f11);
#pragma unroll
      for (int k = 0; k < VEC; ++k) {
        if (c0 + k < a.C) {
          const float top = (1.f - lw) * f00[k] + lw * f01[k];
          const float bot = (1.f - lw) * f10[k] + lw * f11[k];
          o[(long)(c0 + k) * plane] = (1.f - lh) * top + lh * bot;
        }
      }
    }
  }
}

template <typename T>
__global__ __launch_bounds__(RS_THREADS) void upsample_to_nchw_v4_kernel(const ResizeArgs a,
                                                                         float* __restrict__ out) {
  constexpr int VEC = Vec<T>::N;
  const T* __restrict__ X = reinterpret_cast<const T*>(a.x);
  const int wq = a.Wo >> 2;
  const long total = (long)a.N * a.Ho * wq;
  const long plane = (long)a.Ho * a.Wo;
  for (long i = (long)blockIdx.x * RS_THREADS + threadIdx.x; i < total;
       i += (long)gridDim.x * RS_THREADS) {
    long p = i;
    const int wo0 = (int)(p % wq) * 4; p /= wq;
    const int ho = (int)(p % a.Ho);
    const int n = (int)(p / a.Ho);
    int h0, h1; float lh;
    taps(a.sh, ho, a.Hi, a.align, h0, h1, lh);
    int w0[4], w1[4]; float lw[4];
#pragma unroll
    for (int j = 0; j < 4; ++j) taps(a.sw, wo0 + j, a.Wi, a.align, w0[j], w1[j], lw[j]);
    const long base = (long)n * a.Hi * a.Wi;
    const T* r0 = X + (base + (long)h0 * a.Wi) * a.ldx;
    const T* r1 = X + (base + (long)h1 * a.Wi) * a.ldx;
    float* o = out + (long)n * a.C * plane + (long)ho * a.Wo + wo0;
    for (int cv = 0; cv < a.CV; ++cv) {
      const int c0 = cv * VEC;
      float res[4][VEC];
#pragma unroll
      for (int j = 0; j < 4; ++j) {
        float f00[VEC], f01[VEC], f10[VEC], f11[VEC];
        Vec<T>::unpack(ldg16(r0 + (long)w0[j] * a.ldx + c0), f00);
        Vec<T>::unpack(ldg16(r0 + (long)w1[j] * a.ldx + c0), f01);
        Vec<T>::unpack(ldg16(r1 + (long)w0[j] * a.ldx + c0), f10);
        Vec<T>::unpack(ldg16(r1 + (long)w1[j] * a.ldx + c0), f11);
#pragma unroll
        for (int k = 0; k < VEC; ++k) {
          const float top = (1.f - lw[j]) * f00[k] + lw[j] * f01[k];
          const float bot = (1.f - lw[j]) * f10[k] + lw[j] * f11[k];
          res[j][k] = (1.f - lh) * top + lh * bot;
        }
      }
#pragma unroll
      for (int k = 0; k < VEC; ++k) {
        if (c0 + k < a.C)
          *reinterpret_cast<float4*>(o + (long)(c0 + k) * plane) =
              make_float4(res[0][k], res[1][k], res[2][k], res[3][k]);
      }
    }
  }
}

template <typename T>
__global__ __launch_bounds__(RS_THREADS) void upsample_to_nchw_bwd_kernel(
    const ResizeArgs a, const float* __restrict__ gy) {
  constexpr int VEC = Vec<T>::N;
  T* __restrict__ GX = reinterpret_cast<T*>(const_cast<void*>(a.x));
  const long total = (long)a.N * a.Hi * a.Wi;
  const long plane = (long)a.Ho * a.Wo;
  for (long i = (long)blockIdx.x * RS_THREADS + threadIdx.x; i < total;
       i += (long)gridDim.x * RS_THREADS) {
    long p = i;
    const int wi = (int)(p % a.Wi); p /= a.Wi;
    const int hi = (int)(p % a.Hi);
    const int n = (int)(p / a.Hi);
    int hlo, hhi, wlo, whi;
    cand_range(a.sh, hi, a.Ho, a.align, hlo, hhi);
    cand_range(a.sw, wi, a.Wo, a.align, wlo, whi);
    for (int cv = 0; cv < a.CV; ++cv) {
      const int c0 = cv * VEC;
      float acc[VEC];
#pragma unroll
      for (int k = 0; k < VEC; ++k) acc[k] = 0.f;
      for (int ho = hlo; ho <= hhi; ++ho) {
        const float wh = tap_weight(a.sh, ho, a.Hi, a.align, hi);
        if (wh == 0.f) continue;
        for (int wo = wlo; wo <= whi; ++wo) {
          const float ww = tap_weight(a.sw, wo, a.Wi, a.align, wi);
          if (ww == 0.f) continue;
          const float w = wh * ww;
          const float* g = gy + (long)n * a.C * plane + (long)ho * a.Wo + wo;
#pragma unroll
          for (int k = 0; k < VEC; ++k)
            if (c0 + k < a.C) acc[k] = fmaf(w, g[(long)(c0 + k) * plane], acc[k]);
        }
      }
      stg16(GX + (((long)n * a.Hi + hi) * a.Wi + wi) * a.ldx + c0, Vec<T>::pack(acc));
    }
  }
}

template <typename T>
__global__ __launch_bounds__(RS_THREADS) void nchw_to_nhwc_pad_kernel(const float* __restrict__ x,
                                                                      T* __restrict__ y, int N,
                                                                      int Cin, long HW) {
  constexpr int VEC = Vec<T>::N;
  const long total = (long)N * HW;
  for (long i = (long)blockIdx.x * RS_THREADS + threadIdx.x; i < total;
       i += (long)gridDim.x * RS_THREADS) {
    const long n = i / HW, p = i - n * HW;
    float f[VEC];
#pragma unroll
    for (int k = 0; k < VEC; ++k) f[k] = (k < Cin) ? x[(n * Cin + k) * HW + p] : 0.f;
    stg16(y + i * VEC, Vec<T>::pack(f));
  }
}

struct AddUpArgs {
  const void* x; const void* r; void* y;
  const float* sx; const float* tx; const float* sr; const float* tr;
  long ldx, ldr, ldy;
  int N, H, W, C, CV, mode_x, mode_r, shift, post_relu;
};

__device__ __forceinline__ int rs_fast_div(int s, int d, float inv) {
  int q = (int)((float)s * inv);
  if (q * d > s) --q;
  if ((q + 1) * d <= s) ++q;
  return q;
}

template <typename T>
__global__ __launch_bounds__(RS_THREADS) void nearest_add_kernel(const AddUpArgs a) {
  constexpr int VEC = Vec<T>::N;
  const T* __restrict__ X = reinterpret_cast<const T*>(a.x);
  const T* __restrict__ R = reinterpret_cast<const T*>(a.r);
  T* __restrict__ Y = reinterpret_cast<T*>(a.y);
  const int total = a.N * a.H * a.W * a.CV;
  const int Hr = a.H >> a.shift, Wr = a.W >> a.shift;
  const float inv_cv = 1.f / (float)a.CV, inv_w = 1.f / (float)a.W, inv_h = 1.f / (float)a.H;
  for (int i = blockIdx.x * RS_THREADS + threadIdx.x; i < total; i += gridDim.x * RS_THREADS) {
    const int p = rs_fast_div(i, a.CV, inv_cv);
    const int c0 = (i - p * a.CV) * VEC;
    const int t = rs_fast_div(p, a.W, inv_w);
    const int w = p - t * a.W;
    const int n = rs_fast_div(t, a.H, inv_h);
    const int h = t - n * a.H;
    float f[VEC], g[VEC];
    Vec<T>::unpack(ldg16(X + (long)p * a.ldx + c0), f);
    apply_prologue<VEC>(f, a.mode_x, a.sx, a.tx, c0);
    const long pr = ((long)n * Hr + (h >> a.shift)) * Wr + (w >> a.shift);
    Vec<T>::unpack(ldg16(R + pr * a.ldr + c0), g);
    apply_prologue<VEC>(g, a.mode_r, a.sr, a.tr, c0);
#pragma unroll
    for (int k = 0; k < VEC; ++k) {
      f[k] += g[k];
      if (a.post_relu) f[k] = fmaxf(f[k], 0.f);
    }
    stg16(Y + (long)p * a.ldy + c0, Vec<T>::pack(f));
  }
}

template <typename T>
__global__ __launch_bounds__(RS_THREADS) void nearest_sum_bwd_kernel(const AddUpArgs a) {
  constexpr int VEC = Vec<T>::N;
  const T* __restrict__ G = reinterpret_cast<const T*>(a.x);
  T* __restrict__ GR = reinterpret_cast<T*>(a.y);
  const int Hr = a.H >> a.shift, Wr = a.W >> a.shift, f = 1 << a.shift;
  const int total = a.N * Hr * Wr * a.CV;
  const float inv_cv = 1.f / (float)a.CV, inv_w = 1.f / (float)Wr, inv_h = 1.f / (float)Hr;
  for (int i = blockIdx.x * RS_THREADS + threadIdx.x; i < total; i += gridDim.x * RS_THREADS) {
    const int p = rs_fast_div(i, a.CV, inv_cv);
    const int c0 = (i - p * a.CV) * VEC;
    const int t = rs_fast_div(p, Wr, inv_w);
    const int wr = p - t * Wr;
    const int n = rs_fast_div(t, Hr, inv_h);
    const int hr = t - n * Hr;
    float acc[VEC];
#pragma unroll
    for (int k = 0; k < VEC; ++k) acc[k] = 0.f;
    for (int dh = 0; dh < f; ++dh)
      for (int dw = 0; dw < f; ++dw) {
        float g[VEC];
        Vec<T>::unpack(ldg16(G + (((long)n * a.H + (hr << a.shift) + dh) * a.W + (wr << a.shift) + dw) * a.ldx + c0), g);
#pragma unroll
        for (int k = 0; k < VEC; ++k) acc[k] += g[k];
      }
    stg16(GR + (long)p * a.ldy + c0, Vec<T>::pack(acc));
  }
}

static int rs_grid(long total) {
  long g = (total + RS_THREADS - 1) / RS_THREADS;
  if (g > 8192) g = 8192;
  if (g < 1) g = 1;
  return (int)g;
}

static int fill_args(ResizeArgs& a, int dtype, const void* x, long ldx, int N, int Hi, int Wi,
                     int C, void* y, long ldy, int Ho, int Wo, int align, bool need_vec_c) {
  const int vec = dtype == DT_BF16 ? 8 : 4;
  SEG_REQUIRE(dtype == DT_F32 || dtype == DT_BF16, "resize: bad dtype %d", dtype);
  SEG_REQUIRE(ldx % vec == 0 && (!need_vec_c || (C % vec == 0 && ldy % vec == 0)),
              "resize: C/ld must be multiples of %d", vec);
  SEG_REQUIRE(N > 0 && Hi > 0 && Wi > 0 && Ho > 0 && Wo > 0, "resize: empty");
  a.x = x; a.y = y; a.scale = nullptr; a.shift = nullptr; a.chan_mul = nullptr;
  a.ldx = ldx; a.ldy = ldy; a.N = N; a.Hi = Hi; a.Wi = Wi; a.Ho = Ho; a.Wo = Wo; a.C = C;
  a.CV = (C + vec - 1) / vec; a.mode = PRO_NONE; a.align = align;
  a.sh = host_scale(Hi, Ho, align); a.sw = host_scale(Wi, Wo, align);
  return 0;
}

}

extern "C" int seg_bilinear_fwd(int dtype, const void* x, long ldx, int N, int Hi, int Wi, int C,
                                int pro_mode, const float* pro_scale, const float* pro_shift,
                                const float* chan_mul, void* y, long ldy, int Ho, int Wo,
                                int align_corners, void* stream) {
  using namespace seg;
  ResizeArgs a;
  if (fill_args(a, dtype, x, ldx, N, Hi, Wi, C, y, ldy, Ho, Wo, align_corners, true)) return 1;
  SEG_REQUIRE(((pro_mode & PRO_AFFINE) == 0) || (pro_scale && pro_shift),
              "bilinear_fwd: missing scale/shift");
  a.mode = pro_mode; a.scale = pro_scale; a.shift = pro_shift; a.chan_mul = chan_mul;
  const int grid = rs_grid((long)N * Ho * Wo * a.CV);
  if (dtype == DT_BF16)
    hipLaunchKernelGGL((bilinear_fwd_kernel<bf16_t>), dim3(grid), dim3(RS_THREADS), 0,
                       (hipStream_t)stream, a);
  else
    hipLaunchKernelGGL((bilinear_fwd_kernel<float>), dim3(grid), dim3(RS_THREADS), 0,
                       (hipStream_t)stream, a);
  return check_launch("bilinear_fwd");
}

extern "C" int seg_bilinear_bwd(int dtype, void* gx, long ldgx, int N, int Hi, int Wi, int C,
                                const void* gy, long ldgy, int Ho, int Wo, int align_corners,
                                void* stream) {
  using namespace seg;
  ResizeArgs a;
  if (fill_args(a, dtype, gx, ldgx, N, Hi, Wi, C, const_cast<void*>(gy), ldgy, Ho, Wo,
                align_corners, true))
    return 1;
  if ((long)Ho * Wo >= 64L * Hi * Wi) {
    const long nblk = (long)N * Hi * Wi * ((a.CV + RSW_CVB - 1) / RSW_CVB);
    SEG_REQUIRE(nblk < (1L << 31), "bilinear_bwd: too many blocks");
    if (dtype == DT_BF16)
      hipLaunchKernelGGL((bilinear_bwd_wide_kernel<bf16_t>), dim3((unsigned)nblk),
                         dim3(RS_THREADS), 0, (hipStream_t)stream, a);
    else
      hipLaunchKernelGGL((bilinear_bwd_wide_kernel<float>), dim3((unsigned)nblk), dim3(RS_THREADS),
                         0, (hipStream_t)stream, a);
    return check_launch("bilinear_bwd (wide)");
  }
  const int grid = rs_grid((long)N * Hi * Wi * a.CV);
  if (dtype == DT_BF16)
    hipLaunchKernelGGL((bilinear_bwd_kernel<bf16_t>), dim3(grid), dim3(RS_THREADS), 0,
                       (hipStream_t)stream, a);
  else
    hipLaunchKernelGGL((bilinear_bwd_kernel<float>), dim3(grid), dim3(RS_THREADS), 0,
                       (hipStream_t)stream, a);
  return check_launch("bilinear_bwd");
}

extern "C" int seg_upsample_to_nchw(int dtype, const void* x, long ldx, int N, int Hi, int Wi,
                                    int C, float* out, int Ho, int Wo, int align_corners,
                                    void* stream) {
  using namespace seg;
  ResizeArgs a;
  if (fill_args(a, dtype, x, ldx, N, Hi, Wi, C, nullptr, 0, Ho, Wo, align_corners, false)) return 1;
  SEG_REQUIRE(ldx >= (long)a.CV * (dtype == DT_BF16 ? 8 : 4), "upsample_to_nchw: ldx too small");
  if (Wo % 4 == 0 && (reinterpret_cast<uintptr_t>(out) & 15) == 0) {
    const int grid4 = rs_grid((long)N * Ho * (Wo / 4));
    if (dtype == DT_BF16)
      hipLaunchKernelGGL((upsample_to_nchw_v4_kernel<bf16_t>), dim3(grid4), dim3(RS_THREADS), 0,
                         (hipStream_t)stream, a, out);
    else
      hipLaunchKernelGGL((upsample_to_nchw_v4_kernel<float>), dim3(grid4), dim3(RS_THREADS), 0,
                         (hipStream_t)stream, a, out);
    return check_launch("upsample_to_nchw");
  }
  const int grid = rs_grid((long)N * Ho * Wo);
  if (dtype == DT_BF16)
    hipLaunchKernelGGL((upsample_to_nchw_kernel<bf16_t>), dim3(grid), dim3(RS_THREADS), 0,
                       (hipStream_t)stream, a, out);
  else
    hipLaunchKernelGGL((upsample_to_nchw_kernel<float>), dim3(grid), dim3(RS_THREADS), 0,
                       (hipStream_t)stream, a, out);
  return check_launch("upsample_to_nchw");
}

extern "C" int seg_upsample_to_nchw_bwd(int dtype, void* gx, long ldgx, int N, int Hi, int Wi,
                                        int C, const float* gy, int Ho, int Wo, int align_corners,
                                        void* stream) {
  using namespace seg;
  ResizeArgs a;
  if (fill_args(a, dtype, gx, ldgx, N, Hi, Wi, C, nullptr, 0, Ho, Wo, align_corners, false))
    return 1;
  SEG_REQUIRE(ldgx >= (long)a.CV * (dtype == DT_BF16 ? 8 : 4), "upsample_to_nchw_bwd: ld small");
  a.CV = (int)(ldgx / (dtype == DT_BF16 ? 8 : 4));
  const int grid = rs_grid((long)N * Hi * Wi);
  if (dtype == DT_BF16)
    hipLaunchKernelGGL((upsample_to_nchw_bwd_kernel<bf16_t>), dim3(grid), dim3(RS_THREADS), 0,
                       (hipStream_t)stream, a, gy);
  else
    hipLaunchKernelGGL((upsample_to_nchw_bwd_kernel<float>), dim3(grid), dim3(RS_THREADS), 0,
                       (hipStream_t)stream, a, gy);
  return check_launch("upsample_to_nchw_bwd");
}

extern "C" int seg_nchw_to_nhwc_pad(int dtype, const float* x, int N, int Cin, int H, int W,
                                    void* y, void* stream) {
  using namespace seg;
  const int vec = dtype == DT_BF16 ? 8 : 4;
  SEG_REQUIRE(dtype == DT_F32 || dtype == DT_BF16, "nchw_to_nhwc_pad: bad dtype %d", dtype);
  SEG_REQUIRE(Cin >= 1 && Cin <= vec, "nchw_to_nhwc_pad: Cin=%d must be <= %d", Cin, vec);
  const long HW = (long)H * W;
  const int grid = rs_grid((long)N * HW);
  if (dtype == DT_BF16)
    hipLaunchKernelGGL((nchw_to_nhwc_pad_kernel<bf16_t>), dim3(grid), dim3(RS_THREADS), 0,
                       (hipStream_t)stream, x, reinterpret_cast<bf16_t*>(y), N, Cin, HW);
  else
    hipLaunchKernelGGL((nchw_to_nhwc_pad_kernel<float>), dim3(grid), dim3(RS_THREADS), 0,
                       (hipStream_t)stream, x, reinterpret_cast<float*>(y), N, Cin, HW);
  return check_launch("nchw_to_nhwc_pad");
}

extern "C" int seg_nearest_add(int dtype, const void* x, long ldx, int mode_x, const float* sx,
                               const float* tx, const void* r, long ldr, int mode_r,
                               const float* sr, const float* tr, int shift, int post_relu, void* y,
                               long ldy, int N, int H, int W, int C, void* stream) {
  using namespace seg;
  const int vec = dtype == DT_BF16 ? 8 : 4;
  SEG_REQUIRE(dtype == DT_F32 || dtype == DT_BF16, "nearest_add: bad dtype %d", dtype);
  SEG_REQUIRE(C % vec == 0 && ldx % vec == 0 && ldr % vec == 0 && ldy % vec == 0,
              "nearest_add: C/ld must be multiples of %d", vec);
  SEG_REQUIRE(shift >= 0 && shift < 8 && (H % (1 << shift)) == 0 && (W % (1 << shift)) == 0,
              "nearest_add: H=%d W=%d not divisible by 2^%d", H, W, shift);
  SEG_REQUIRE((long)N * H * W * (C / vec) < (1L << 31), "nearest_add: too large");
  AddUpArgs a;
  a.x = x; a.r = r; a.y = y; a.sx = sx; a.tx = tx; a.sr = sr; a.tr = tr;
  a.ldx = ldx; a.ldr = ldr; a.ldy = ldy; a.N = N; a.H = H; a.W = W; a.C = C; a.CV = C / vec;
  a.mode_x = mode_x; a.mode_r = mode_r; a.shift = shift; a.post_relu = post_relu;
  const int grid = rs_grid((long)N * H * W * a.CV);
  if (dtype == DT_BF16)
    hipLaunchKernelGGL((nearest_add_kernel<bf16_t>), dim3(grid), dim3(RS_THREADS), 0, (hipStream_t)stream, a);
  else
    hipLaunchKernelGGL((nearest_add_kernel<float>), dim3(grid), dim3(RS_THREADS), 0, (hipStream_t)stream, a);
  return check_launch("nearest_add");
}

extern "C" int seg_nearest_sum_bwd(int dtype, const void* g, long ldg, int N, int H, int W, int C,
                                   int shift, void* gr, long ldgr, void* stream) {
  using namespace seg;
  const int vec = dtype == DT_BF16 ? 8 : 4;
  SEG_REQUIRE(dtype == DT_F32 || dtype == DT_BF16, "nearest_sum_bwd: bad dtype %d", dtype);
  SEG_REQUIRE(C % vec == 0 && ldg % vec == 0 && ldgr % vec == 0, "nearest_sum_bwd: C/ld");
  SEG_REQUIRE(shift >= 0 && shift < 8 && (H % (1 << shift)) == 0 && (W % (1 << shift)) == 0,
              "nearest_sum_bwd: size not divisible");
  AddUpArgs a;
  a.x = g; a.r = nullptr; a.y = gr; a.sx = a.tx = a.sr = a.tr = nullptr;
  a.ldx = ldg; a.ldr = 0; a.ldy = ldgr; a.N = N; a.H = H; a.W = W; a.C = C; a.CV = C / vec;
  a.mode_x = 0; a.mode_r = 0; a.shift = shift; a.post_relu = 0;
  const int grid = rs_grid((long)N * (H >> shift) * (W >> shift) * a.CV);
  if (dtype == DT_BF16)
    hipLaunchKernelGGL((nearest_sum_bwd_kernel<bf16_t>), dim3(grid), dim3(RS_THREADS), 0, (hipStream_t)stream, a);
  else
    hipLaunchKernelGGL((nearest_sum_bwd_kernel<float>), dim3(grid), dim3(RS_THREADS), 0, (hipStream_t)stream, a);
  return check_launch("nearest_sum_bwd");
}
```

Measured before the change: 89.60 images/sec.

## Extend sliding-window depthwise conv to dilation 2 and add row-blocked bilinear kernels

The sliding-window depthwise 3x3 kernel now handles dilation up to 2 by splitting rows into dilation phases, so each phase runs as a dense stride-1 slide over every d-th row with column taps offset by d. Blocks with no rows write zero partials so the reduction layout stays fixed. Bilinear forward and backward gain row-blocked kernels, on by default, in which each block covers one output or input row segment and threads split channels, replacing the flat per-element grid. This is meant to cut redundant index and weight math and improve locality, at the cost of extra geometry paths and a new dilated code path that must stay correct.

```diff
diff --git a/include/segmentron_hip.h b/include/segmentron_hip.h
--- a/include/segmentron_hip.h
+++ b/include/segmentron_hip.h
@@ -29,6 +29,7 @@
                   const float* pro_scale, const float* pro_shift, void* y, long ldy, int Ho, int Wo,
                   float* stat_partial, int grid_y, void* stream);
 int seg_dwconv_grid_y(int dtype, int C, int N, int Ho, int Wo, int stride, int dil, int kind);
+int seg_dw_slide_max_dil(int v);
 int seg_dwconv3x3_wgrad_finalize(const float* partial, int R, int C, float* dw_c9, void* stream);
 int seg_dwconv3x3_wgrad(int dtype, const void* x, long ldx, int N, int Hi, int Wi, int C,
                         const void* dy, long lddy, int Ho, int Wo, int stride, int dil,
@@ -155,6 +156,14 @@
                      void* stream);
 int seg_bilinear_bwd(int dtype, void* gx, long ldgx, int N, int Hi, int Wi, int C, const void* gy,
                      long ldgy, int Ho, int Wo, int align_corners, void* stream);
+int seg_bilinear_rows(int v);
+int seg_bilinear_fwd_flat(int dtype, const void* x, long ldx, int N, int Hi, int Wi, int C,
+                          int pro_mode, const float* pro_scale, const float* pro_shift,
+                          const float* chan_mul, void* y, long ldy, int Ho, int Wo,
+                          int align_corners, void* stream);
+int seg_bilinear_bwd_flat(int dtype, void* gx, long ldgx, int N, int Hi, int Wi, int C,
+                          const void* gy, long ldgy, int Ho, int Wo, int align_corners,
+                          void* stream);
 int seg_nearest_add(int dtype, const void* x, long ldx, int mode_x, const float* sx,
                     const float* tx, const void* r, long ldr, int mode_r, const float* sr,
                     const float* tr, int shift, int post_relu, void* y, long ldy, int N, int H,
diff --git a/segmentron_amd/csrc/dwconv.hip b/segmentron_amd/csrc/dwconv.hip
--- a/segmentron_amd/csrc/dwconv.hip
+++ b/segmentron_amd/csrc/dwconv.hip
@@ -431,8 +431,8 @@
                                  int kind) {
   using namespace seg;
   const int tiled_stride = kind == 0 ? stride : 1;
-  if ((kind == 0 || kind == 1) && dw_slide_supported(stride, dil, C))
-    return dw_slide_rows(C, N, Ho, Wo);
+  if ((kind == 0 || kind == 1) && dw_slide_supported(stride, dil, C, N, Ho, Wo))
+    return dw_slide_rows(C, N, Ho, Wo, dil);
   if ((kind == 0 || stride == 1) && dw_tiled_supported(tiled_stride, dil))
     return dw_tiled_grid_y(dtype, C, N, Ho, Wo, kind);
   if (kind == 0 && stride == 2 && dil == 1)
@@ -451,6 +451,8 @@
   if (gy > cap) gy = cap;
   return (int)gy;
 }
+extern "C" int seg_dw_slide_max_dil(int v) { return seg::dw_slide_max_dil(v); }
+
 extern "C" int seg_dwconv3x3(int dtype, int mode, const void* x, long ldx, int N, int Hi, int Wi,
                              int C, const float* w9c, int w_layout, int stride, int dil, int pro_mode,
                              const float* pro_scale, const float* pro_shift, void* y, long ldy,
@@ -464,9 +466,9 @@
               "dwconv3x3: affine prologue without scale/shift");
   SEG_REQUIRE(mode == MODE_FWD || stat_partial == nullptr, "dwconv3x3: stats only in forward");
   SEG_REQUIRE(grid_y >= 1, "dwconv3x3: grid_y must be >= 1");
-  if (mode == MODE_FWD && dw_slide_supported(stride, dil, C)) {
+  if (mode == MODE_FWD && dw_slide_supported(stride, dil, C, N, Hi, Wi)) {
     SEG_REQUIRE(Ho == Hi && Wo == Wi, "dwconv3x3: stride 1 keeps the size");
-    return launch_dw_slide_fwd(dtype, x, ldx, N, Hi, Wi, C, w9c, w_layout, pro_mode, pro_scale,
+    return launch_dw_slide_fwd(dtype, x, ldx, N, Hi, Wi, C, w9c, w_layout, dil, pro_mode, pro_scale,
                                pro_shift, y, ldy, stat_partial, grid_y, (hipStream_t)stream);
   }
   if (mode == MODE_FWD && dw_tiled_supported(stride, dil)) {
@@ -564,8 +566,8 @@
   SEG_REQUIRE(((pro_mode & PRO_AFFINE) == 0) || (pro_scale && pro_shift),
               "dwconv3x3_bwd_fused_add: affine prologue without scale/shift");
   SEG_REQUIRE(grid_y >= 1 && partial_w != nullptr, "dwconv3x3_bwd_fused_add: bad grid/partials");
-  if (dw_slide_supported(1, 1, C))
-    return launch_dw_slide_bwd(dtype, dy, lddy, x, ldx, N, H, W, C, w9c, w_layout, pro_mode,
+  if (dw_slide_supported(1, 1, C, N, H, W))
+    return launch_dw_slide_bwd(dtype, dy, lddy, x, ldx, N, H, W, C, w9c, w_layout, 1, pro_mode,
                                pro_scale, pro_shift, g, ldg, partial_w, partial_bn, grid_y,
                                (hipStream_t)stream, res, ldr);
   return launch_dw_bwd_tiled(dtype, dy, lddy, x, ldx, N, H, W, C, w9c, w_layout, 1, pro_mode,
@@ -587,8 +589,8 @@
   SEG_REQUIRE(((pro_mode & PRO_AFFINE) == 0) || (pro_scale && pro_shift),
               "dwconv3x3_bwd_fused: affine prologue without scale/shift");
   SEG_REQUIRE(grid_y >= 1 && partial_w != nullptr, "dwconv3x3_bwd_fused: bad grid/partials");
-  if (dw_slide_supported(1, dil, C))
-    return launch_dw_slide_bwd(dtype, dy, lddy, x, ldx, N, H, W, C, w9c, w_layout, pro_mode,
+  if (dw_slide_supported(1, dil, C, N, H, W))
+    return launch_dw_slide_bwd(dtype, dy, lddy, x, ldx, N, H, W, C, w9c, w_layout, dil, pro_mode,
                                pro_scale, pro_shift, g, ldg, partial_w, partial_bn, grid_y,
                                (hipStream_t)stream);
   if (dw_tiled_supported(1, dil)) {
diff --git a/segmentron_amd/csrc/dwconv_slide.h b/segmentron_amd/csrc/dwconv_slide.h
--- a/segmentron_amd/csrc/dwconv_slide.h
+++ b/segmentron_amd/csrc/dwconv_slide.h
@@ -2,14 +2,16 @@
 #include <hip/hip_runtime.h>
 
 namespace seg {
-bool dw_slide_supported(int stride, int dil, int C);
-int dw_slide_rows(int C, int N, int H, int W);
+bool dw_slide_supported(int stride, int dil, int C, int N, int H, int W);
+int dw_slide_max_dil(int v);
+int dw_slide_rows(int C, int N, int H, int W, int dil);
 int launch_dw_slide_fwd(int dtype, const void* x, long ldx, int N, int H, int W, int C,
-                        const float* w, int w_layout, int pro_mode, const float* sc,
+                        const float* w, int w_layout, int dil, int pro_mode, const float* sc,
                         const float* sh, void* y, long ldy, float* stat_partial, int rows,
                         hipStream_t st);
 int launch_dw_slide_bwd(int dtype, const void* dy, long lddy, const void* x, long ldx, int N, int H,
-                        int W, int C, const float* w, int w_layout, int pro_mode, const float* sc,
-                        const float* sh, void* g, long ldg, float* partial_w, float* partial_bn,
-                        int rows, hipStream_t st, const void* res = nullptr, long ldr = 0);
+                        int W, int C, const float* w, int w_layout, int dil, int pro_mode,
+                        const float* sc, const float* sh, void* g, long ldg, float* partial_w,
+                        float* partial_bn, int rows, hipStream_t st, const void* res = nullptr,
+                        long ldr = 0);
 }
diff --git a/segmentron_amd/csrc/dwconv_slide.hip b/segmentron_amd/csrc/dwconv_slide.hip
--- a/segmentron_amd/csrc/dwconv_slide.hip
+++ b/segmentron_amd/csrc/dwconv_slide.hip
@@ -20,9 +20,10 @@
   float* partial_bn;
   long ldx, lddy, ldy, ldr;
   int N, H, W, C, pro_mode, rs, nstrips, nwblk, ncblk;
+  int dil, spp;
 };
 
-struct SlBlock { int n, strip, wblk, cblk, prow; };
+struct SlBlock { int n, ph, strip, wblk, cblk, prow; };
 __device__ __forceinline__ SlBlock sl_block(const DwSlideArgs& a) {
   const int nblk = a.ncblk * a.nwblk * a.nstrips * a.N;
   int L = xcd_remap(blockIdx.x, nblk);
@@ -32,8 +33,10 @@
   b.prow = L;
   b.wblk = L % a.nwblk;
   L /= a.nwblk;
-  b.strip = L % a.nstrips;
+  const int s = L % a.nstrips;
   b.n = L / a.nstrips;
+  b.ph = s / a.spp;
+  b.strip = s - b.ph * a.spp;
   return b;
 }
 
@@ -138,7 +141,7 @@
 }
 
 struct SlThread {
-  int c, w, r0, r1, rlast;
+  int c, w, r0, r1, rlast, hp;
   bool live, lm, rm;
   unsigned off_m, off_0, off_p;
   bool edge, first, last;
@@ -153,14 +156,16 @@
   t.c = min(cfull, a.C - 4);
   t.w = min(wfull, a.W - 1);
   t.live = wfull < a.W && cfull < a.C;
-  t.lm = t.w >= 1;
-  t.rm = t.w + 1 < a.W;
+  const int d = a.dil;
+  t.lm = t.w >= d;
+  t.rm = t.w + d < a.W;
+  t.hp = b.ph < a.H ? (a.H - b.ph + d - 1) / d : 0;
   t.r0 = b.strip * a.rs;
-  t.r1 = min(a.H, t.r0 + a.rs);
-  t.rlast = min(t.r1, a.H - 1);
-  t.off_m = (unsigned)((max(t.w - 1, 0) * ld + t.c) * ESIZE);
+  t.r1 = min(t.hp, t.r0 + a.rs);
+  t.rlast = min(t.r1, t.hp - 1);
+  t.off_m = (unsigned)((max(t.w - d, 0) * ld + t.c) * ESIZE);
   t.off_0 = (unsigned)((t.w * ld + t.c) * ESIZE);
-  t.off_p = (unsigned)((min(t.w + 1, a.W - 1) * ld + t.c) * ESIZE);
+  t.off_p = (unsigned)((min(t.w + d, a.W - 1) * ld + t.c) * ESIZE);
   const int lane = tid & 63, col = lane >> 4;
   t.first = col == 0;
   t.last = col == 3;
@@ -232,12 +237,12 @@
 
   Q4 wt[9], sc, sh;
   sc = sh = q4_zero();
-  const unsigned char* __restrict__ Xb = reinterpret_cast<const unsigned char*>(a.x) +
-                                         (long)b.n * a.H * a.W * a.ldx * ES;
-  unsigned char* __restrict__ Yb = reinterpret_cast<unsigned char*>(a.y) +
-                                   (long)b.n * a.H * a.W * a.ldy * ES;
-  const long xpitch = (long)a.W * a.ldx * ES, ypitch = (long)a.W * a.ldy * ES;
-  const unsigned rowbytes = (unsigned)xpitch;
+  const long xrow = (long)a.W * a.ldx * ES, yrow = (long)a.W * a.ldy * ES;
+  const long prow0 = (long)b.n * a.H + b.ph;
+  const unsigned char* __restrict__ Xb = reinterpret_cast<const unsigned char*>(a.x) + prow0 * xrow;
+  unsigned char* __restrict__ Yb = reinterpret_cast<unsigned char*>(a.y) + prow0 * yrow;
+  const long xpitch = xrow * a.dil, ypitch = yrow * a.dil;
+  const unsigned rowbytes = (unsigned)xrow;
   const unsigned yoff = t.live ? (unsigned)((t.w * a.ldy + t.c) * ES) : 0xFFFFFFFFu;
 
   auto issue = [&](int r, raw_t (&raw)[3]) {
@@ -253,7 +258,7 @@
   };
   auto commit = [&](int r, const raw_t (&raw)[3], Q4 (&row)[3], auto check) {
     constexpr bool CHECK = decltype(check)::value;
-    const bool rv = !CHECK || (r >= 0 && r < a.H);
+    const bool rv = !CHECK || (r >= 0 && r < t.hp);
     raw_t r3[3];
     r3[1] = raw[0];
     if (XCHG) {
@@ -278,12 +283,19 @@
     for (int kw = 0; kw < 3; ++kw) q4_fma(acc, rb[kw], wt[3 + kw]);
 #pragma unroll
     for (int kw = 0; kw < 3; ++kw) q4_fma(acc, rc[kw], wt[6 + kw]);
-    sl_st_row<raw_t>(Yb + (long)ro * ypitch, (unsigned)ypitch, yoff, IO::pack(acc));
+    sl_st_row<raw_t>(Yb + (long)ro * ypitch, (unsigned)yrow, yoff, IO::pack(acc));
     ssum.lo += acc.lo; ssum.hi += acc.hi;
     q4_fma(ssq, acc, acc);
   };
 
   constexpr int D = SL_DEPTH_F, U = (D % 3 == 0) ? D : 3 * D;
+  if (r0 >= r1) {
+    if (a.partial != nullptr && tid < SL_CQ * 8) {
+      const int ch = (b.cblk * SL_CQ + (tid >> 3)) * 4 + (tid & 3);
+      if (ch < a.C) a.partial[((long)b.prow * 2 + ((tid & 7) >> 2)) * a.C + ch] = 0.f;
+    }
+    return;
+  }
   Q4 win[3][3];
   raw_t ring[D][3];
 #pragma unroll
@@ -359,15 +371,16 @@
 
   Q4 wt[9], sc, sh;
   sc = sh = q4_zero();
-  const long img = (long)b.n * a.H * a.W;
+  const long img = ((long)b.n * a.H + b.ph) * a.W;
   const unsigned char* __restrict__ Db = reinterpret_cast<const unsigned char*>(a.dy) + img * a.lddy * ES;
   const unsigned char* __restrict__ Xb = reinterpret_cast<const unsigned char*>(a.x) + img * a.ldx * ES;
   const unsigned char* __restrict__ Rb =
       RES ? reinterpret_cast<const unsigned char*>(a.res) + img * a.ldr * ES : nullptr;
   unsigned char* __restrict__ Gb = reinterpret_cast<unsigned char*>(a.y) + img * a.ldy * ES;
-  const long dpitch = (long)a.W * a.lddy * ES, xpitch = (long)a.W * a.ldx * ES;
-  const long rpitch = (long)a.W * a.ldr * ES, gpitch = (long)a.W * a.ldy * ES;
-  const unsigned rowbytes = (unsigned)dpitch;
+  const long drow = (long)a.W * a.lddy * ES, grow = (long)a.W * a.ldy * ES;
+  const long dpitch = drow * a.dil, xpitch = (long)a.W * a.ldx * ES * a.dil;
+  const long rpitch = (long)a.W * a.ldr * ES * a.dil, gpitch = grow * a.dil;
+  const unsigned rowbytes = (unsigned)drow;
   const unsigned xoff = (unsigned)((t.w * a.ldx + t.c) * ES), roff = (unsigned)((t.w * a.ldr + t.c) * ES);
   const unsigned goff = t.live ? (unsigned)((t.w * a.ldy + t.c) * ES) : 0xFFFFFFFFu;
 
@@ -389,7 +402,7 @@
   };
   auto commit = [&](int r, const raw_t (&raw)[3], Q4 (&row)[3], auto check) {
     constexpr bool CHECK = decltype(check)::value;
-    const bool rv = !CHECK || (r >= 0 && r < a.H);
+    const bool rv = !CHECK || (r >= 0 && r < t.hp);
     raw_t r3[3];
     r3[1] = raw[0];
     if (XCHG) {
@@ -430,15 +443,26 @@
       Q4 o;
       o.lo = g.lo + rr.lo;
       o.hi = g.hi + rr.hi;
-      sl_st_row<raw_t>(Gb + (long)ro * gpitch, (unsigned)gpitch, goff, IO::pack(o));
+      sl_st_row<raw_t>(Gb + (long)ro * gpitch, (unsigned)grow, goff, IO::pack(o));
     } else {
-      sl_st_row<raw_t>(Gb + (long)ro * gpitch, (unsigned)gpitch, goff, IO::pack(g));
+      sl_st_row<raw_t>(Gb + (long)ro * gpitch, (unsigned)grow, goff, IO::pack(g));
     }
     s1.lo += g.lo; s1.hi += g.hi;
     q4_fma(s2, g, xr);
   };
 
   constexpr int D = SL_DEPTH_B, U = (D % 3 == 0) ? D : 3 * D;
+  if (r0 >= r1) {
+    for (int e = tid; e < SL_CQ * 44; e += SL_THREADS) {
+      const int q = e / 44, k = e - q * 44;
+      const int ch = (b.cblk * SL_CQ + q) * 4 + (k & 3), r = k >> 2;
+      if (ch < a.C) {
+        if (r < 9) a.partial[((long)b.prow * 9 + r) * a.C + ch] = 0.f;
+        else if (a.partial_bn != nullptr) a.partial_bn[((long)b.prow * 2 + (r - 9)) * a.C + ch] = 0.f;
+      }
+    }
+    return;
+  }
   Q4 win[3][3];
   raw_t ring[D][3], xring[D], rring[D];
 #pragma unroll
@@ -521,31 +545,45 @@
   }
 }
 
-bool dw_slide_supported(int stride, int dil, int C) { return stride == 1 && dil == 1 && C % 4 == 0; }
-
-static void slide_geom(DwSlideArgs& a, int N, int H, int W, int C) {
+static int g_slide_max_dil = 2;
+int dw_slide_max_dil(int v) {
+  const int old = g_slide_max_dil;
+  if (v >= 1) g_slide_max_dil = v;
+  return old;
+}
+
+bool dw_slide_supported(int stride, int dil, int C, int N, int H, int W) {
+  if (stride != 1 || dil < 1 || dil > g_slide_max_dil || C % 4 != 0) return false;
+  (void)H;
+  return dil == 1 || (long)N * dil * ((W + SL_WL - 1) / SL_WL) <= 1024;
+}
+
+static void slide_geom(DwSlideArgs& a, int N, int H0, int W, int C, int dil) {
   a.ncblk = (C / 4 + SL_CQ - 1) / SL_CQ;
   a.nwblk = (W + SL_WL - 1) / SL_WL;
+  a.dil = dil;
+  const int H = (H0 + dil - 1) / dil;
   long ns = (H + 21) / 43;
-  const long per_strip = (long)N * a.nwblk * a.ncblk;
+  const long per_strip = (long)N * a.nwblk * a.ncblk * dil;
   const long want = (400 + per_strip - 1) / per_strip;
   if (ns < want) ns = want;
   if (ns > H / 8) ns = H / 8;
-  const long cap = 1024 / ((long)N * a.nwblk);
+  const long cap = 1024 / ((long)N * a.nwblk * dil);
   if (ns > cap) ns = cap;
   if (ns < 1) ns = 1;
   a.rs = (int)((H + ns - 1) / ns);
-  a.nstrips = (H + a.rs - 1) / a.rs;
-}
-
-int dw_slide_rows(int C, int N, int H, int W) {
+  a.spp = (H + a.rs - 1) / a.rs;
+  a.nstrips = a.spp * dil;
+}
+
+int dw_slide_rows(int C, int N, int H, int W, int dil) {
   DwSlideArgs a;
-  slide_geom(a, N, H, W, C);
+  slide_geom(a, N, H, W, C, dil);
   return N * a.nstrips * a.nwblk;
 }
 
 static bool slide_exchange(const DwSlideArgs& a, int esize) {
-  return (long)a.N * a.H * a.W * a.C * esize >= (30L << 20);
+  return a.dil == 1 && (long)a.N * a.H * a.W * a.C * esize >= (30L << 20);
 }
 template <typename T>
 static void slide_launch_fwd(const DwSlideArgs& a, dim3 grid, hipStream_t st) {
@@ -578,7 +616,7 @@
 static bool slide_mode_ok(int m) { return m == 0 || m == 1 || m == 2 || m == 3 || m == 5 || m == 7; }
 
 int launch_dw_slide_fwd(int dtype, const void* x, long ldx, int N, int H, int W, int C,
-                        const float* w, int w_layout, int pro_mode, const float* sc,
+                        const float* w, int w_layout, int dil, int pro_mode, const float* sc,
                         const float* sh, void* y, long ldy, float* stat_partial, int rows,
                         hipStream_t st) {
   DwSlideArgs a;
@@ -586,7 +624,7 @@
   a.sc = sc; a.sh = sh; a.partial = stat_partial; a.partial_bn = nullptr;
   a.ldx = ldx; a.lddy = 0; a.ldy = ldy; a.ldr = 0;
   a.N = N; a.H = H; a.W = W; a.C = C; a.pro_mode = pro_mode;
-  slide_geom(a, N, H, W, C);
+  slide_geom(a, N, H, W, C, dil);
   SEG_REQUIRE(slide_mode_ok(pro_mode), "dwconv (slide): unsupported prologue mode %d", pro_mode);
   SEG_REQUIRE(C % 4 == 0 && ldx % 4 == 0 && ldy % 4 == 0,
               "dwconv (slide): C/ldx/ldy must be multiples of 4");
@@ -600,15 +638,15 @@
 }
 
 int launch_dw_slide_bwd(int dtype, const void* dy, long lddy, const void* x, long ldx, int N, int H,
-                        int W, int C, const float* w, int w_layout, int pro_mode, const float* sc,
-                        const float* sh, void* g, long ldg, float* partial_w, float* partial_bn,
-                        int rows, hipStream_t st, const void* res, long ldr) {
+                        int W, int C, const float* w, int w_layout, int dil, int pro_mode,
+                        const float* sc, const float* sh, void* g, long ldg, float* partial_w,
+                        float* partial_bn, int rows, hipStream_t st, const void* res, long ldr) {
   DwSlideArgs a;
   a.x = x; a.dy = dy; a.res = res; a.y = g; a.w = w; a.w_layout = w_layout & 1;
   a.sc = sc; a.sh = sh; a.partial = partial_w; a.partial_bn = partial_bn;
   a.ldx = ldx; a.lddy = lddy; a.ldy = ldg; a.ldr = ldr;
   a.N = N; a.H = H; a.W = W; a.C = C; a.pro_mode = pro_mode;
-  slide_geom(a, N, H, W, C);
+  slide_geom(a, N, H, W, C, dil);
   SEG_REQUIRE(slide_mode_ok(pro_mode), "dwconv bwd (slide): unsupported prologue mode %d", pro_mode);
   SEG_REQUIRE(C % 4 == 0 && ldx % 4 == 0 && lddy % 4 == 0 && ldg % 4 == 0 &&
                   (res == nullptr || ldr % 4 == 0),
diff --git a/segmentron_amd/csrc/resize.hip b/segmentron_amd/csrc/resize.hip
--- a/segmentron_amd/csrc/resize.hip
+++ b/segmentron_amd/csrc/resize.hip
@@ -12,6 +12,7 @@
   int N, Hi, Wi, Ho, Wo, C, CV;
   int mode, align;
   float sh, sw;
+  int lp_log2, nseg, segw;
 };
 
 template <typename T>
@@ -94,6 +95,104 @@
   }
 }
 
+template <typename T>
+__global__ __launch_bounds__(RS_THREADS) void bilinear_fwd_rows_kernel(const ResizeArgs a) {
+  constexpr int VEC = Vec<T>::N;
+  const T* __restrict__ X = reinterpret_cast<const T*>(a.x);
+  T* __restrict__ Y = reinterpret_cast<T*>(a.y);
+  const int row = blockIdx.x / a.nseg, seg = blockIdx.x - row * a.nseg;
+  const int n = row / a.Ho, ho = row - n * a.Ho;
+  int h0, h1; float lh;
+  taps(a.sh, ho, a.Hi, a.align, h0, h1, lh);
+  const T* __restrict__ r0 = X + ((long)n * a.Hi + h0) * a.Wi * a.ldx;
+  const T* __restrict__ r1 = X + ((long)n * a.Hi + h1) * a.Wi * a.ldx;
+  T* __restrict__ yr = Y + ((long)n * a.Ho + ho) * a.Wo * a.ldy;
+  const int lp = 1 << a.lp_log2, pp = RS_THREADS >> a.lp_log2;
+  const int cl = threadIdx.x & (lp - 1), ps = threadIdx.x >> a.lp_log2;
+  const int wend = min((seg + 1) * a.segw, a.Wo);
+  for (int wo = seg * a.segw + ps; wo < wend; wo += pp) {
+    int w0, w1; float lw;
+    taps(a.sw, wo, a.Wi, a.align, w0, w1, lw);
+    const T* __restrict__ p00 = r0 + (long)w0 * a.ldx;
+    const T* __restrict__ p01 = r0 + (long)w1 * a.ldx;
+    const T* __restrict__ p10 = r1 + (long)w0 * a.ldx;
+    const T* __restrict__ p11 = r1 + (long)w1 * a.ldx;
+    T* __restrict__ py = yr + (long)wo * a.ldy;
+    for (int cv = cl; cv < a.CV; cv += lp) {
+      const int c0 = cv * VEC;
+      const uint4 q00 = ldg16(p00 + c0), q01 = ldg16(p01 + c0);
+      const uint4 q10 = ldg16(p10 + c0), q11 = ldg16(p11 + c0);
+      float f00[VEC], f01[VEC], f10[VEC], f11[VEC];
+      Vec<T>::unpack(q00, f00);
+      Vec<T>::unpack(q01, f01);
+      Vec<T>::unpack(q10, f10);
+      Vec<T>::unpack(q11, f11);
+      apply_prologue<VEC>(f00, a.mode, a.scale, a.shift, c0);
+      apply_prologue<VEC>(f01, a.mode, a.scale, a.shift, c0);
+      apply_prologue<VEC>(f10, a.mode, a.scale, a.shift, c0);
+      apply_prologue<VEC>(f11, a.mode, a.scale, a.shift, c0);
+      float o[VEC];
+#pragma unroll
+      for (int k = 0; k < VEC; ++k) {
+        const float top = (1.f - lw) * f00[k] + lw * f01[k];
+        const float bot = (1.f - lw) * f10[k] + lw * f11[k];
+        o[k] = (1.f - lh) * top + lh * bot;
+      }
+      if (a.chan_mul) {
+        const float* m = a.chan_mul + (long)n * a.C + c0;
+#pragma unroll
+        for (int k = 0; k < VEC; ++k) o[k] *= m[k];
+      }
+      stg16(py + c0, Vec<T>::pack(o));
+    }
+  }
+}
+
+template <typename T>
+__global__ __launch_bounds__(RS_THREADS) void bilinear_bwd_rows_kernel(const ResizeArgs a) {
+  constexpr int VEC = Vec<T>::N;
+  const T* __restrict__ GY = reinterpret_cast<const T*>(a.y);
+  T* __restrict__ GX = reinterpret_cast<T*>(const_cast<void*>(a.x));
+  const int row = blockIdx.x / a.nseg, seg = blockIdx.x - row * a.nseg;
+  const int n = row / a.Hi, hi = row - n * a.Hi;
+  int hlo, hhi;
+  cand_range(a.sh, hi, a.Ho, a.align, hlo, hhi);
+  while (hlo < hhi && tap_weight(a.sh, hlo, a.Hi, a.align, hi) == 0.f) ++hlo;
+  while (hhi > hlo && tap_weight(a.sh, hhi, a.Hi, a.align, hi) == 0.f) --hhi;
+  const int lp = 1 << a.lp_log2;
+  const int cl = threadIdx.x & (lp - 1), ps = threadIdx.x >> a.lp_log2;
+  const int wfull = seg * a.segw + ps;
+  const bool live = wfull < a.Wi;
+  const int wi = min(wfull, a.Wi - 1);
+  int wlo, whi;
+  cand_range(a.sw, wi, a.Wo, a.align, wlo, whi);
+  while (wlo < whi && tap_weight(a.sw, wlo, a.Wi, a.align, wi) == 0.f) ++wlo;
+  while (whi > wlo && tap_weight(a.sw, whi, a.Wi, a.align, wi) == 0.f) --whi;
+  const T* __restrict__ gimg = GY + (long)n * a.Ho * a.Wo * a.ldy;
+  T* __restrict__ px = GX + (((long)n * a.Hi + hi) * a.Wi + wi) * a.ldx;
+  for (int cv = cl; cv < a.CV; cv += lp) {
+    const int c0 = cv * VEC;
+    float acc[VEC];
+#pragma unroll
+    for (int k = 0; k < VEC; ++k) acc[k] = 0.f;
+    for (int ho = hlo; ho <= hhi; ++ho) {
+      const float wh = tap_weight(a.sh, ho, a.Hi, a.align, hi);
+      const T* __restrict__ grow = gimg + (long)ho * a.Wo * a.ldy + c0;
+      for (int wo = wlo; wo <= whi; ++wo) {
+        const uint4 q = ldg16(grow + (long)wo * a.ldy);
+        const float ww = tap_weight(a.sw, wo, a.Wi, a.align, wi);
+        const bool use = wh != 0.f && ww != 0.f;
+        const float w = wh * ww;
+        float g[VEC];
+        Vec<T>::unpack(q, g);
+#pragma unroll
+        for (int k = 0; k < VEC; ++k) acc[k] = use ? fmaf(w, g[k], acc[k]) : acc[k];
+      }
+    }
+    if (live) stg16(px + c0, Vec<T>::pack(acc));
+  }
+}
+
 constexpr int RSW_CVB = 8, RSW_PL = RS_THREADS / RSW_CVB;
 template <typename T>
 __global__ __launch_bounds__(RS_THREADS) void bilinear_bwd_wide_kernel(const ResizeArgs a) {
@@ -375,21 +474,45 @@
   a.ldx = ldx; a.ldy = ldy; a.N = N; a.Hi = Hi; a.Wi = Wi; a.Ho = Ho; a.Wo = Wo; a.C = C;
   a.CV = (C + vec - 1) / vec; a.mode = PRO_NONE; a.align = align;
   a.sh = host_scale(Hi, Ho, align); a.sw = host_scale(Wi, Wo, align);
+  a.lp_log2 = 0; a.nseg = 1; a.segw = 0;
   return 0;
 }
 
-}
-
-extern "C" int seg_bilinear_fwd(int dtype, const void* x, long ldx, int N, int Hi, int Wi, int C,
-                                int pro_mode, const float* pro_scale, const float* pro_shift,
-                                const float* chan_mul, void* y, long ldy, int Ho, int Wo,
-                                int align_corners, void* stream) {
-  using namespace seg;
+static long rows_geom(ResizeArgs& a, long rows, int W, int passes) {
+  a.lp_log2 = 0;
+  while ((1 << a.lp_log2) < a.CV && (1 << a.lp_log2) < RS_THREADS) ++a.lp_log2;
+  a.segw = (RS_THREADS >> a.lp_log2) * passes;
+  a.nseg = (W + a.segw - 1) / a.segw;
+  return rows * a.nseg;
+}
+
+static int g_bilinear_rows = 1;
+static int bilinear_rows(int v) {
+  const int old = g_bilinear_rows;
+  if (v >= 0) g_bilinear_rows = v != 0;
+  return old;
+}
+
+static int bilinear_fwd_host(bool flat, int dtype, const void* x, long ldx, int N, int Hi, int Wi,
+                             int C, int pro_mode, const float* pro_scale, const float* pro_shift,
+                             const float* chan_mul, void* y, long ldy, int Ho, int Wo,
+                             int align_corners, void* stream) {
   ResizeArgs a;
   if (fill_args(a, dtype, x, ldx, N, Hi, Wi, C, y, ldy, Ho, Wo, align_corners, true)) return 1;
   SEG_REQUIRE(((pro_mode & PRO_AFFINE) == 0) || (pro_scale && pro_shift),
               "bilinear_fwd: missing scale/shift");
   a.mode = pro_mode; a.scale = pro_scale; a.shift = pro_shift; a.chan_mul = chan_mul;
+  if (!flat) {
+    const long nblk = rows_geom(a, (long)N * Ho, Wo, 8);
+    SEG_REQUIRE(nblk < (1L << 31), "bilinear_fwd: too many blocks");
+    if (dtype == DT_BF16)
+      hipLaunchKernelGGL((bilinear_fwd_rows_kernel<bf16_t>), dim3((unsigned)nblk), dim3(RS_THREADS),
+                         0, (hipStream_t)stream, a);
+    else
+      hipLaunchKernelGGL((bilinear_fwd_rows_kernel<float>), dim3((unsigned)nblk), dim3(RS_THREADS),
+                         0, (hipStream_t)stream, a);
+    return check_launch("bilinear_fwd");
+  }
   const int grid = rs_grid((long)N * Ho * Wo * a.CV);
   if (dtype == DT_BF16)
     hipLaunchKernelGGL((bilinear_fwd_kernel<bf16_t>), dim3(grid), dim3(RS_THREADS), 0,
@@ -397,18 +520,17 @@
   else
     hipLaunchKernelGGL((bilinear_fwd_kernel<float>), dim3(grid), dim3(RS_THREADS), 0,
                        (hipStream_t)stream, a);
-  return check_launch("bilinear_fwd");
-}
-
-extern "C" int seg_bilinear_bwd(int dtype, void* gx, long ldgx, int N, int Hi, int Wi, int C,
-                                const void* gy, long ldgy, int Ho, int Wo, int align_corners,
-                                void* stream) {
-  using namespace seg;
+  return check_launch("bilinear_fwd (flat)");
+}
+
+static int bilinear_bwd_host(bool flat, bool test_flat, int dtype, void* gx, long ldgx, int N, int Hi, int Wi, int C,
+                             const void* gy, long ldgy, int Ho, int Wo, int align_corners,
+                             void* stream) {
   ResizeArgs a;
   if (fill_args(a, dtype, gx, ldgx, N, Hi, Wi, C, const_cast<void*>(gy), ldgy, Ho, Wo,
                 align_corners, true))
     return 1;
-  if ((long)Ho * Wo >= 64L * Hi * Wi) {
+  if (!test_flat && (long)Ho * Wo >= 64L * Hi * Wi) {
     const long nblk = (long)N * Hi * Wi * ((a.CV + RSW_CVB - 1) / RSW_CVB);
     SEG_REQUIRE(nblk < (1L << 31), "bilinear_bwd: too many blocks");
     if (dtype == DT_BF16)
@@ -419,6 +541,17 @@
                          0, (hipStream_t)stream, a);
     return check_launch("bilinear_bwd (wide)");
   }
+  if (!flat) {
+    const long nblk = rows_geom(a, (long)N * Hi, Wi, 1);
+    SEG_REQUIRE(nblk < (1L << 31), "bilinear_bwd: too many blocks");
+    if (dtype == DT_BF16)
+      hipLaunchKernelGGL((bilinear_bwd_rows_kernel<bf16_t>), dim3((unsigned)nblk), dim3(RS_THREADS),
+                         0, (hipStream_t)stream, a);
+    else
+      hipLaunchKernelGGL((bilinear_bwd_rows_kernel<float>), dim3((unsigned)nblk), dim3(RS_THREADS),
+                         0, (hipStream_t)stream, a);
+    return check_launch("bilinear_bwd");
+  }
   const int grid = rs_grid((long)N * Hi * Wi * a.CV);
   if (dtype == DT_BF16)
     hipLaunchKernelGGL((bilinear_bwd_kernel<bf16_t>), dim3(grid), dim3(RS_THREADS), 0,
@@ -426,7 +559,37 @@
   else
     hipLaunchKernelGGL((bilinear_bwd_kernel<float>), dim3(grid), dim3(RS_THREADS), 0,
                        (hipStream_t)stream, a);
-  return check_launch("bilinear_bwd");
+  return check_launch("bilinear_bwd (flat)");
+}
+
+}
+
+extern "C" int seg_bilinear_fwd(int dtype, const void* x, long ldx, int N, int Hi, int Wi, int C,
+                                int pro_mode, const float* pro_scale, const float* pro_shift,
+                                const float* chan_mul, void* y, long ldy, int Ho, int Wo,
+                                int align_corners, void* stream) {
+  return seg::bilinear_fwd_host(!seg::g_bilinear_rows, dtype, x, ldx, N, Hi, Wi, C, pro_mode, pro_scale, pro_shift,
+                                chan_mul, y, ldy, Ho, Wo, align_corners, stream);
+}
+extern "C" int seg_bilinear_bwd(int dtype, void* gx, long ldgx, int N, int Hi, int Wi, int C,
+                                const void* gy, long ldgy, int Ho, int Wo, int align_corners,
+                                void* stream) {
+  return seg::bilinear_bwd_host(!seg::g_bilinear_rows, false, dtype, gx, ldgx, N, Hi, Wi, C, gy, ldgy, Ho, Wo,
+                                align_corners, stream);
+}
+extern "C" int seg_bilinear_rows(int v) { return seg::bilinear_rows(v); }
+extern "C" int seg_bilinear_fwd_flat(int dtype, const void* x, long ldx, int N, int Hi, int Wi,
+                                     int C, int pro_mode, const float* pro_scale,
+                                     const float* pro_shift, const float* chan_mul, void* y,
+                                     long ldy, int Ho, int Wo, int align_corners, void* stream) {
+  return seg::bilinear_fwd_host(true, dtype, x, ldx, N, Hi, Wi, C, pro_mode, pro_scale, pro_shift,
+                                chan_mul, y, ldy, Ho, Wo, align_corners, stream);
+}
+extern "C" int seg_bilinear_bwd_flat(int dtype, void* gx, long ldgx, int N, int Hi, int Wi, int C,
+                                     const void* gy, long ldgy, int Ho, int Wo, int align_corners,
+                                     void* stream) {
+  return seg::bilinear_bwd_host(true, true, dtype, gx, ldgx, N, Hi, Wi, C, gy, ldgy, Ho, Wo,
+                                align_corners, stream);
 }
 
 extern "C" int seg_upsample_to_nchw(int dtype, const void* x, long ldx, int N, int Hi, int Wi,
```

New measurement: 90.12 images/sec, median of 6. Within noise of the previous version (+0.6%).
